# akashsengupta1997/HierarchicalProbabilistic3DHuman

Measured on AMD Instinct MI355X. Metric: images/sec end-to-end (num_samples=100), higher is better.
Workload: dtype f32

## Files before the change

hierarchicalprobabilistic3dhuman_amd/_capi.py:

```python
import contextlib
import ctypes
import os

import torch

_PKG_DIR = os.path.dirname(os.path.abspath(__file__))
LIB_PATH = os.path.join(_PKG_DIR, "libhps.so")
DEV_LIB_PATH = os.path.join(_PKG_DIR, "libhps_dev.so")

_c = ctypes
_P = _c.c_void_p
_I = _c.c_int

_PROTOTYPES = {
    "hps_version": [],
    "hps_last_error": [],
    "hps_stream_create_cu_partition": [_I, _I, _c.POINTER(_P)],
    "hps_stream_destroy": [_P],
    "hps_smpl_pose_prep": [_P, _P, _I, _P, _I, _P, _P, _P, _P, _I, _P, _I, _I, _P, _P, _P, _I, _P],
    "hps_smpl_blend": [_P, _P, _P, _P, _I, _I, _I, _I, _I, _I, _P],
    "hps_smpl_lbs": [_P, _I, _P, _P, _P, _I, _I, _P, _P, _I, _I, _P],
    "hps_smpl_mesh_fused": [_P, _P, _P, _P, _P, _P, _I, _I, _P, _P, _I, _I, _I, _I, _I, _P],
    "hps_smpl_mesh_fused_picks": [_P, _P, _P, _P, _P, _P, _I, _I, _P, _P, _I, _I, _I, _I, _I, _P, _P, _I, _P],
    "hps_smpl_mesh_fused_shared_shape": [_P] * 8 + [_I, _I, _P] + [_I] * 5 + [_P, _P, _I, _P],
    "hps_smpl_split_bf16x3_bytes": [_I, _I],
    "hps_smpl_split_bf16x3_mesh_tile": [],
    "hps_smpl_split_bf16x3": [_P, _I, _I, _I, _I, _P, _P],
    "hps_smpl_mesh_fused_shared_shape_bf16x3": [_P] * 8 + [_I, _I, _P] + [_I] * 4 + [_P, _P, _I, _P],
    "hps_smpl_v_shaped": [_P, _I, _P, _I, _P, _P, _I, _I, _P],
    "hps_smpl_mesh_fused_np": [_I],
    "hps_smpl_lbs_backward": [_P, _I, _P, _P, _P, _I, _I, _P, _P, _I, _P, _P, _P, _P, _P, _P, _I, _I, _P],
    "hps_smpl_blend_backward": [_P, _P, _P, _P, _I, _I, _I, _I, _I, _P],
    "hps_smpl_pose_prep_backward": [_P, _P, _I, _P, _I, _P, _P, _P, _P, _I, _P, _P, _I, _P, _I, _P, _P, _P, _I, _P],
    "hps_smpl_joints": [_P, _P, _P, _P, _P, _I, _I, _P, _P, _I, _I, _P],
    "hps_vertex_uncertainty": [_P, _P, _I, _I, _I, _P],
    "hps_joints_and_uncertainty": [_P, _P, _P, _P, _P, _I, _I, _P, _P, _I, _I, _P, _P, _I, _I, _I, _P],
    "hps_query_workspace": [_I, _c.c_int64, _c.c_int64, _c.c_int64],
    "hps_mf_sample": [_P, _P, _P, _P, _P, _I, _I, _I, _I, _c.c_float, _c.c_float, _P, _P, _P, _c.c_uint64,
                      _c.c_int64, _P, _I, _P, _P, _P, _P],
    "hps_infer_assemble": [_P, _P, _P, _P, _P, _P, _P, _I, _I, _I, _I, _P],
    "hps_quat_to_rotmat": [_P, _P, _I, _P],
    "hps_rot6d_to_rotmat": [_P, _P, _I, _P],
    "hps_batch_rodrigues": [_P, _P, _I, _P],
    "hps_linear": [_P, _I, _P, _P, _P, _P, _I, _I, _I, _I, _I, _P],
    "hps_head_trunk": [_P] + [_I] + [_P] * 14 + [_I] * 7 + [_P],
    "hps_head_joint_level": [_P, _I, _I, _P, _I, _P, _P, _P, _P, _P, _P, _P, _P, _P, _c.c_float, _P, _P, _I, _I, _P],
    "hps_head_joint_level_svd": [_P, _I, _I, _P, _I, _P, _P, _P, _P, _P, _P, _P, _P, _P, _c.c_float, _P, _P, _P, _P, _I, _I, _I, _P],
    "hps_svd3_packed": [_P, _P, _I, _I, _P],
    "hps_host_svd3_emulated": [_P, _P, _I, _I],
    "hps_host_svd_flavor": [],
    "hps_host_svd3_packed": [_P, _P, _I, _I],
    "hps_host_bind_lapack": [_c.c_char_p],
    "hps_head_svd_finish": [_P, _P, _I, _P, _P, _P, _P, _P, _P, _I, _I, _P],
    "hps_canny_edges": [_P, _P, _I, _P, _P, _P, _P, _P, _P, _I, _I, _I, _I, _c.c_float, _I, _P],
    "hps_canny_edge_map": [_P, _P, _I, _P, _c.c_int64, _I, _I, _I, _I, _c.c_float, _I, _P],
    "hps_proxy_rep": [_P, _P, _P, _P, _I, _I, _I, _I, _c.c_float, _P],
    "hps_pointset_errors": [_P, _P, _I, _I, _I, _I, _P, _P, _P, _P, _P],
    "hps_heatmaps_to_joints2d": [_P, _P, _P, _I, _I, _I, _c.c_float, _P],
    "hps_sample_joints2d_error": [_P, _P, _I, _P, _P, _P, _c.c_float, _P, _I, _I, _P],
    "hps_conv2d_bn_act_pad": [_P, _P, _P, _P, _P, _P, _I, _I, _I, _I, _I, _I, _I, _I, _I, _I, _I, _I, _I, _I, _I, _P, _P],
    "hps_conv2d_bn_act_pad_down": [_P] * 9 + [_I] * 14 + [_P, _P],
    "hps_conv3x3_winograd": [_P, _P, _P, _P, _P, _P, _I, _I, _I, _I, _I, _I, _I, _I, _P, _P],
    "hps_conv3x3_winograd_workspace": [_I, _I, _I, _I, _I],
    "hps_stem_phase_frames_bytes": [_I, _I, _I],
    "hps_stem_phase_split": [_P, _P, _I, _I, _I, _I, _P],
    "hps_proxy_rep_phase_frames": [_P, _P, _P, _P, _I, _I, _I, _I, _c.c_float, _P],
    "hps_stem_winograd": [_P, _P, _P, _P, _P, _I, _I, _I, _I, _I, _P],
    "hps_stem_pool_side_bytes": [_I, _I, _I],
    "hps_stem_winograd_pooled": [_P, _P, _P, _P, _P, _P, _I, _I, _I, _I, _I, _P],
    "hps_stem_winograd_pooled_nchw": [_P, _P, _P, _P, _P, _P, _I, _I, _I, _I, _I, _P],
    "hps_sums_f64": [_P, _P, _P, _I, _c.c_double, _P, _P, _P, _P],
    "hps_sizeof_enc_op": [],
    "hps_encoder_run": [_P, _I, _P],
    "hps_head_pose_levels": [_P, _I, _I, _P, _P, _I, _P, _P, _P, _P, _P, _P, _P, _P, _P, _c.c_float, _P, _P, _P, _P, _P, _P,
                             _P, _P, _I, _I, _I, _I, _P],
    "hps_nchw_to_padded_nhwc": [_P, _P, _I, _I, _I, _I, _I, _P],
    "hps_nchw_to_padded_nhwc_generic": [_P, _P, _I, _I, _I, _I, _I, _I, _I, _P],
    "hps_maxpool3x3s2_pad": [_P, _P, _I, _I, _I, _I, _I, _P],
    "hps_global_avgpool_pad": [_P, _P, _I, _I, _I, _I, _I, _P],
    "hps_mf_log_norm_const": [_P, _I, _P, _P, _P, _P],
    "hps_mf_nll": [_P, _P, _P, _P, _P, _I, _c.c_double, _P, _P, _P, _P, _P],
    "hps_mf_loss_forward": [_P, _P, _P, _P],
    "hps_mf_loss_backward": [_P, _P, _P, _P],
    "hps_head_forward_refine": [_P, _I] + [_P] * 9 + [_I] + [_P] * 6 + [_c.c_float] + [_P] * 13 + [_I] * 7 + [_P],
    "hps_head_pose_levels_backward": [_P, _I, _I, _P, _P, _I] + [_P] * 21 + [_I, _I, _I, _P],
    "hps_head_pose_levels_backward_factors": [_P, _I, _I, _P, _P, _I] + [_P] * 23 + [_I, _I, _I, _P],
    "hps_mf_sample_keep_quat": [_P, _P, _P, _I, _I, _I, _I, _c.c_float, _c.c_float, _P, _P, _P, _c.c_uint64, _c.c_int64, _I, _P, _P, _P, _P],
    "hps_mf_sample_backward": [_P, _P, _P, _P, _P, _P, _P, _P, _I, _I, _I, _c.c_float, _P, _P, _P, _P],
    "hps_head_trunk_backward": [_P, _I] + [_P] * 20 + [_I] * 7 + [_P],
    "hps_rot6d_to_rotmat_backward": [_P, _P, _P, _I, _P],
    "hps_conv_wgrad": [_P] * 4 + [_I] * 12 + [_P],
    "hps_conv_wgrad_slice_pixels": [_I, _I],
    "hps_conv_wgrad_workspace": [_I] * 9,
    "hps_conv_dgrad": [_P] * 4 + [_I] * 12 + [_P],
    "hps_relu_gate_pad": [_P] * 4 + [_I] * 6 + [_P],
    "hps_relu_gate_workspace": [_I] * 4,
    "hps_maxpool3x3s2_backward": [_P] * 3 + [_I] * 5 + [_P],
    "hps_global_avgpool_backward": [_P] * 2 + [_I] * 5 + [_P],
    "hps_bn_batch_stats": [_P] * 4 + [_I] * 5 + [_P],
    "hps_bn_batch_stats_workspace": [_I] * 4,
    "hps_bn_train_fold": [_P] * 5 + [_c.c_double, _c.c_double, _c.c_longlong] + [_P] * 5 + [_I, _P],
    "hps_bn_apply_act_pad": [_P] * 5 + [_I] * 7 + [_P],
    "hps_bn_train_backward_sums": [_P] * 7 + [_I] * 7 + [_P],
    "hps_bn_train_backward_sums_workspace": [_I] * 4,
    "hps_bn_train_backward_dz": [_P] * 7 + [_I] * 7 + [_P],
    "hps_seg_bbox_affine": [_P, _c.c_int64, _P, _I, _I, _I, _I, _c.c_float, _P, _P, _P, _P, _P, _P],
    "hps_train_crop_augment": [_P, _c.c_int64, _P, _P, _P, _P, _I, _I, _I, _I, _I, _P, _P, _P, _P, _P],
    "hps_train_joints2d": [_P, _P, _P, _P, _P, _I, _I, _c.c_float, _I, _I, _P, _P, _P, _P, _P],
}
_RESTYPES = {"hps_last_error": _c.c_char_p, "hps_smpl_split_bf16x3_bytes": _c.c_size_t, "hps_query_workspace": _c.c_int64, "hps_conv3x3_winograd_workspace": _c.c_size_t,
             "hps_stem_phase_frames_bytes": _c.c_size_t, "hps_stem_pool_side_bytes": _c.c_size_t,
             "hps_conv_wgrad_workspace": _c.c_size_t, "hps_relu_gate_workspace": _c.c_size_t,
             "hps_bn_batch_stats_workspace": _c.c_size_t, "hps_bn_train_backward_sums_workspace": _c.c_size_t}

EXPORTED_SYMBOLS = tuple(_PROTOTYPES)

_lib = None
_dev_lib = None
_use_dev = False


class EncOp(_c.Structure):
    _fields_ = [("kind", _I), ("x", _P), ("w", _P), ("scale", _P), ("shift", _P), ("residual", _P), ("y", _P),
                ("splitk_ws", _P)] + [(n, _I) for n in ("B", "H", "W", "ipad", "Cin", "Cout", "KH", "KW", "stride", "pad", "opad",
                                                       "relu", "row_mode", "variant", "ksplit")] + [
                    ("w_down", _P), ("scale_down", _P), ("shift_down", _P), ("y_down", _P)]


class MfLossArgs(_c.Structure):
    _fields_ = [("struct_bytes", _I), ("reduction", _I)] + [
        (n, _c.c_int64) for n in ("n_pose", "shape_B", "n_shape", "j2d_B", "Ns", "K", "n_glob", "n_verts", "n_joints3d")] + [
        ("img_wh", _c.c_double), ("overreg", _c.c_double), ("weights", _c.c_double * 6)] + [
        (n, _P) for n in ("pose_F", "pose_U", "pose_S", "pose_V", "shape_loc", "shape_scale", "joints2d", "glob_rotmats", "verts",
                          "joints3d", "t_pose_rotmats", "t_shape", "t_joints2d", "t_joints2d_vis", "t_glob_rotmats", "t_verts",
                          "t_joints3d", "g_pose_F", "g_pose_S", "g_shape_loc", "g_shape_scale", "g_joints2d", "g_glob_rotmats",
                          "g_verts", "g_joints3d")]


MF_REDUCTION_MEAN, MF_REDUCTION_SUM = 0, 1
ENC_RELAYOUT, ENC_CONV, ENC_MAXPOOL, ENC_AVGPOOL, ENC_CONV_WINOGRAD, ENC_STEM_SPLIT, ENC_STEM_WINOGRAD, ENC_RELAYOUT_GENERIC = 0, 1, 2, 3, 4, 5, 6, 7
ENC_STEM_WINOGRAD_POOLED, ENC_STEM_WINOGRAD_POOLED_NCHW, ENC_CONV_DOWN = 8, 9, 10
ENC_ENTRY = {kind: (entry, tuple(fields.split())) for kind, entry, fields in (
    (ENC_RELAYOUT, "hps_nchw_to_padded_nhwc", "x y B Cin H W opad"),
    (ENC_RELAYOUT_GENERIC, "hps_nchw_to_padded_nhwc_generic", "x y B Cin Cout H W KW opad"),
    (ENC_CONV, "hps_conv2d_bn_act_pad", "x w scale shift residual y B H W ipad Cin Cout KH KW stride pad opad relu row_mode variant ksplit splitk_ws"),
    (ENC_CONV_DOWN, "hps_conv2d_bn_act_pad_down", "x w scale shift y w_down scale_down shift_down y_down B H W ipad Cin Cout KH KW stride pad opad "
                                                  "relu variant ksplit splitk_ws"),
    (ENC_CONV_WINOGRAD, "hps_conv3x3_winograd", "x w scale shift residual y B H W ipad Cin Cout opad relu splitk_ws"),
    (ENC_STEM_SPLIT, "hps_stem_phase_split", "x y B Cin H W"),
    (ENC_STEM_WINOGRAD, "hps_stem_winograd", "x w scale shift y B H W opad relu"),
    (ENC_STEM_WINOGRAD_POOLED, "hps_stem_winograd_pooled", "x w scale shift y splitk_ws B H W opad relu"),
    (ENC_STEM_WINOGRAD_POOLED_NCHW, "hps_stem_winograd_pooled_nchw", "x w scale shift y splitk_ws B H W opad relu"),
    (ENC_MAXPOOL, "hps_maxpool3x3s2_pad", "x y B H W Cin opad"),
    (ENC_AVGPOOL, "hps_global_avgpool_pad", "x y B H W Cin ipad"))}
SVD_HOST, SVD_DEVICE, SVD_DEVICE_FMA = 0, 1, 2
SVD_ROUNDING_REFERENCE, SVD_ROUNDING_FMA = 0, 1
HEAD_WIDE_WORKGROUPS = 0x100


class HpsError(RuntimeError):
    pass


def _open(path, prototypes, what):
    if not os.path.exists(path):
        raise HpsError(
            "%s is missing (%s). Build it with `python -m hierarchicalprobabilistic3dhuman_amd.build` "
            "(hipcc --offload-arch=gfx950). There is no CPU fallback for this path." % (what, path))
    lib = ctypes.CDLL(path)
    for name, argtypes in prototypes.items():
        fn = getattr(lib, name)
        fn.argtypes = argtypes
        fn.restype = _RESTYPES.get(name, _I)
    torch_cpu = os.path.join(os.path.dirname(torch.__file__), "lib", "libtorch_cpu.so")
    if os.path.exists(torch_cpu):
        lib.hps_host_bind_lapack(torch_cpu.encode())
    return lib


def load(dev=False):
    global _lib, _dev_lib
    if dev:
        if _dev_lib is None:
            _dev_lib = _open(DEV_LIB_PATH, dict(_PROTOTYPES, **_dev_prototypes()), "libhps_dev.so")
        return _dev_lib
    if _lib is None:
        _lib = _open(LIB_PATH, _PROTOTYPES, "libhps.so")
    return _lib


def _dev_prototypes():
    import importlib.util
    path = os.path.join(os.path.dirname(_PKG_DIR), "tests", "devlib.py")
    if not os.path.exists(path):
        raise HpsError("libhps_dev.so is test infrastructure: its prototypes live in tests/devlib.py, which is missing (%s)" % path)
    spec = importlib.util.spec_from_file_location("hps_tests_devlib_prototypes", path)
    mod = importlib.util.module_from_spec(spec)
    spec.loader.exec_module(mod)
    return mod.DEV_PROTOTYPES


@contextlib.contextmanager
def dev_library():
    global _use_dev
    prev, _use_dev = _use_dev, True
    try:
        yield load(dev=True)
    finally:
        _use_dev = prev


def require_device(t, what="tensor"):
    if not isinstance(t, torch.Tensor) or not t.is_cuda:
        raise HpsError(
            "%s must live on a HIP (MI355X) device; this package has no CPU path "
            "(the CPU oracle under oracle/ is test infrastructure only)" % what)
    if t.device.index != torch.cuda.current_device():
        raise HpsError("%s lives on cuda:%d but the current device is cuda:%d; call torch.cuda.set_device(%d) "
                       "(or use `with torch.cuda.device(...)`) before calling into libhps"
                       % (what, t.device.index, torch.cuda.current_device(), t.device.index))


def ptr(t, dtype=torch.float32, what="tensor"):
    if t is None:
        return None
    require_device(t, what)
    if t.dtype != dtype:
        raise HpsError("%s: expected %s, got %s" % (what, dtype, t.dtype))
    if not t.is_contiguous():
        raise HpsError("%s must be contiguous" % what)
    return _P(t.data_ptr())


def iptr(t, what="index tensor"):
    return ptr(t, torch.int32, what)


def stream():
    return _P(torch.cuda.current_stream().cuda_stream)


def cu_partition_stream(first_cu, num_cus):
    s = _P()
    call("hps_stream_create_cu_partition", int(first_cu), int(num_cus), _c.byref(s))
    if not _partition_streams:
        import atexit
        atexit.register(_destroy_partition_streams)
    _partition_streams.append(s.value)
    return torch.cuda.ExternalStream(s.value)


_partition_streams = []


def _destroy_partition_streams():
    try:
        if torch.cuda.is_available():
            torch.cuda.synchronize()
        lib = load()
        while _partition_streams:
            lib.hps_stream_destroy(_P(_partition_streams.pop()))
    except Exception:
        pass


_svd_flavor = None
_svd_flavor_exact = None


def svd_flavor():
    global _svd_flavor, _svd_flavor_exact
    if _svd_flavor is None:
        fl = load(dev=_use_dev).hps_host_svd_flavor()
        _svd_flavor_exact = fl in (SVD_ROUNDING_REFERENCE, SVD_ROUNDING_FMA)
        if not _svd_flavor_exact:
            import warnings
            warnings.warn("libhps: neither rounding flavour of the in-kernel 3x3 SVD reproduces this host's LAPACK sgesdd bit for "
                          "bit; using reference rounding (expect about one differently signed singular-vector pair in 10^4 "
                          "matrices relative to torch.svd on this host; svd_mode='host' is exact)")
            fl = SVD_ROUNDING_REFERENCE
        _svd_flavor = fl
    return _svd_flavor


def svd_flavor_is_exact():
    svd_flavor()
    return bool(_svd_flavor_exact)


def call(name, *args):
    lib = load(dev=_use_dev)
    rc = getattr(lib, name)(*args)
    if rc != 0:
        msg = lib.hps_last_error()
        raise HpsError("%s failed (code %d): %s" % (name, rc, msg.decode() if msg else ""))


def issue_enc_op(op):
    entry, fields = ENC_ENTRY[op.kind]
    call(entry, *[getattr(op, f) for f in fields], stream())


def run_enc_ops(ops, first, count, composite=True):
    if not composite:
        for i in range(first, first + count):
            issue_enc_op(ops[i])
    elif first == 0:
        call("hps_encoder_run", ops, count, stream())
    else:
        call("hps_encoder_run", _c.cast(_c.byref(ops, first * _c.sizeof(EncOp)), _c.POINTER(EncOp)), count, stream())


WS_CONV_SPLITK, WS_SMPL_MP, WS_SMPL_XT, WS_SMPL_A, WS_SMPL_VPOSED, WS_HEAD_F, WS_HEAD_USV = range(7)
WS_MF_LOSS = 8
WS_SMPL_LBS_BWD, WS_SMPL_BLEND_BWD = 9, 10
WS_HEAD_LEVELS_BWD, WS_HEAD_TRUNK_BWD = 11, 12
WS_SEG_BBOX = 13


def query_workspace(what, d0=0, d1=0, d2=0):
    n = load(dev=_use_dev).hps_query_workspace(int(what), int(d0), int(d1), int(d2))
    if n < 0:
        raise HpsError("hps_query_workspace(%d, %d, %d, %d) failed" % (what, d0, d1, d2))
    return int(n)


def f32c(t):
    if t.dtype != torch.float32:
        t = t.float()
    return t.contiguous()
```

hierarchicalprobabilistic3dhuman_amd/csrc/composite.hip:

```cpp
#include <vector>

#include "hps_common.h"

using namespace hps;

extern "C" int hps_sizeof_enc_op(void) { return (int)sizeof(hps_enc_op); }

extern "C" int hps_encoder_run(const hps_enc_op* ops, int n_ops, hps_stream_t stream) {
    if (!ops && n_ops > 0) return bad_arg("hps_encoder_run: null op list");
    for (int i = 0; i < n_ops; ++i) {
        const hps_enc_op& o = ops[i];
        int rc;
        switch (o.kind) {
            case HPS_ENC_RELAYOUT:
                rc = hps_nchw_to_padded_nhwc(o.x, o.y, o.B, o.Cin, o.H, o.W, o.opad, stream);
                break;
            case HPS_ENC_RELAYOUT_GENERIC:
                rc = hps_nchw_to_padded_nhwc_generic(o.x, o.y, o.B, o.Cin, o.Cout, o.H, o.W, o.KW, o.opad, stream);
                break;
            case HPS_ENC_CONV:
                rc = hps_conv2d_bn_act_pad(o.x, o.w, o.scale, o.shift, o.residual, o.y, o.B, o.H, o.W, o.ipad, o.Cin, o.Cout,
                                           o.KH, o.KW, o.stride, o.pad, o.opad, o.relu, o.row_mode, o.variant, o.ksplit,
                                           o.splitk_ws, stream);
                break;
            case HPS_ENC_CONV_DOWN:
                rc = hps_conv2d_bn_act_pad_down(o.x, o.w, o.scale, o.shift, o.y, o.w_down, o.scale_down, o.shift_down, o.y_down, o.B, o.H,
                                                o.W, o.ipad, o.Cin, o.Cout, o.KH, o.KW, o.stride, o.pad, o.opad, o.relu, o.variant, o.ksplit,
                                                o.splitk_ws, stream);
                break;
            case HPS_ENC_CONV_WINOGRAD:
                rc = hps_conv3x3_winograd(o.x, o.w, o.scale, o.shift, o.residual, o.y, o.B, o.H, o.W, o.ipad, o.Cin, o.Cout, o.opad,
                                          o.relu, o.splitk_ws, stream);
                break;
            case HPS_ENC_STEM_SPLIT:
                rc = hps_stem_phase_split(o.x, o.y, o.B, o.Cin, o.H, o.W, stream);
                break;
            case HPS_ENC_STEM_WINOGRAD:
                rc = hps_stem_winograd(o.x, o.w, o.scale, o.shift, o.y, o.B, o.H, o.W, o.opad, o.relu, stream);
                break;
            case HPS_ENC_STEM_WINOGRAD_POOLED:
                rc = hps_stem_winograd_pooled(o.x, o.w, o.scale, o.shift, o.y, o.splitk_ws, o.B, o.H, o.W, o.opad, o.relu, stream);
                break;
            case HPS_ENC_STEM_WINOGRAD_POOLED_NCHW:
                rc = hps_stem_winograd_pooled_nchw(o.x, o.w, o.scale, o.shift, o.y, o.splitk_ws, o.B, o.H, o.W, o.opad, o.relu, stream);
                break;
            case HPS_ENC_MAXPOOL:
                rc = hps_maxpool3x3s2_pad(o.x, o.y, o.B, o.H, o.W, o.Cin, o.opad, stream);
                break;
            case HPS_ENC_AVGPOOL:
                rc = hps_global_avgpool_pad(o.x, o.y, o.B, o.H, o.W, o.Cin, o.ipad, stream);
                break;
            default:
                return bad_arg("hps_encoder_run: unknown op kind");
        }
        if (rc != HPS_OK) return rc;
    }
    return HPS_OK;
}

extern "C" int hps_head_pose_levels(const float* embed, int embed_dim, int hidden, const int32_t* level_joints,
                                    const int32_t* level_sizes_host, int n_levels, const int32_t* anc_ptr,
                                    const int32_t* anc_idx, const float* const* w1t_ptrs, const float* const* b1_ptrs,
                                    const float* const* w2_ptrs, const float* const* b2_ptrs, float* u_proper,
                                    float* s_proper, float* mode, float delta_i_weight, float* pose_f, float* pose_u,
                                    float* pose_s, float* pose_v, float* f_level_dev, float* usv_level_dev,
                                    float* f_host_pinned, float* usv_host_pinned, int B, int num_body_joints,
                                    int svd_threads, int svd_mode, hps_stream_t stream) {
    if (!embed || !level_joints || !level_sizes_host) return bad_arg("hps_head_pose_levels: null pointer");
    const int wide = svd_mode & HPS_HEAD_WIDE_WORKGROUPS;
    svd_mode &= ~HPS_HEAD_WIDE_WORKGROUPS;
    if (svd_mode == HPS_SVD_DEVICE || svd_mode == HPS_SVD_DEVICE_FMA) {
        const int flavor = (svd_mode == HPS_SVD_DEVICE_FMA ? HPS_SVD_ROUNDING_FMA : HPS_SVD_ROUNDING_REFERENCE) | wide;
        int first_d = 0;
        for (int l = 0; l < n_levels; ++l) {
            const int n_level = level_sizes_host[l];
            const int rc = hps_head_joint_level_svd(embed, embed_dim, hidden, level_joints + first_d, n_level, anc_ptr, anc_idx,
                                                    w1t_ptrs, b1_ptrs, w2_ptrs, b2_ptrs, u_proper, s_proper, mode, delta_i_weight,
                                                    pose_f, pose_u, pose_s, pose_v, B, num_body_joints, flavor, stream);
            if (rc != HPS_OK) return rc;
            first_d += n_level;
        }
        return HPS_OK;
    }
    if (svd_mode != HPS_SVD_HOST) return bad_arg("hps_head_pose_levels: svd_mode");
    if (!f_level_dev || !usv_level_dev || !f_host_pinned || !usv_host_pinned)
        return bad_arg("hps_head_pose_levels: the host-LAPACK mode needs the staging buffers");
    hipStream_t s = (hipStream_t)stream;
    int first = 0;
    for (int l = 0; l < n_levels; ++l) {
        const int n_level = level_sizes_host[l];
        const int32_t* ids = level_joints + first;
        const size_t count = (size_t)B * n_level;
        int rc = hps_head_joint_level(embed, embed_dim, hidden, ids, n_level, anc_ptr, anc_idx, w1t_ptrs, b1_ptrs, w2_ptrs,
                                      b2_ptrs, u_proper, s_proper, mode, delta_i_weight, pose_f, f_level_dev, B,
                                      num_body_joints, stream);
        if (rc != HPS_OK) return rc;
        hipError_t e = hipMemcpyAsync(f_host_pinned, f_level_dev, count * 9 * sizeof(float), hipMemcpyDeviceToHost, s);
        if (e == hipSuccess) e = hipStreamSynchronize(s);
        if (e != hipSuccess) {
            set_error("hps_head_pose_levels: %s", hipGetErrorString(e));
            return (int)e;
        }
        rc = hps_host_svd3_packed(f_host_pinned, usv_host_pinned, (int)count, svd_threads);
        if (rc != HPS_OK) return rc;
        e = hipMemcpyAsync(usv_level_dev, usv_host_pinned, count * 21 * sizeof(float), hipMemcpyHostToDevice, s);
        if (e != hipSuccess) {
            set_error("hps_head_pose_levels: %s", hipGetErrorString(e));
            return (int)e;
        }
        rc = hps_head_svd_finish(usv_level_dev, ids, n_level, pose_u, pose_s, pose_v, u_proper, s_proper, mode, B,
                                 num_body_joints, stream);
        if (rc != HPS_OK) return rc;
        first += n_level;
    }
    return HPS_OK;
}
```

hierarchicalprobabilistic3dhuman_amd/csrc/head.hip:

```cpp
#include "hps_common.h"
#include "svd3_gesdd.h"

namespace hps {

__device__ __forceinline__ float elu1(float x) { return x > 0.0f ? x : expm1f(x); }


constexpr int TB = 8;
constexpr int LCOLS = 16;
constexpr int LKS = 16;

template <int ROWS>
__device__ __forceinline__ void dot_slice(const float* __restrict__ w, size_t ldw, const float* xs, int k_lo, int k_hi,
                                          float (&acc)[ROWS]) {
    int k = k_lo;
    for (; k + 8 <= k_hi; k += 8) {
        float wv[8];
#pragma unroll
        for (int u = 0; u < 8; ++u) wv[u] = w[(size_t)(k + u) * ldw];
#pragma unroll
        for (int u = 0; u < 8; ++u) {
            const float4* xr = reinterpret_cast<const float4*>(xs + (k + u) * ROWS);
#pragma unroll
            for (int q = 0; q < ROWS / 4; ++q) {
                const float4 xv = xr[q];
                acc[q * 4 + 0] += xv.x * wv[u]; acc[q * 4 + 1] += xv.y * wv[u];
                acc[q * 4 + 2] += xv.z * wv[u]; acc[q * 4 + 3] += xv.w * wv[u];
            }
        }
    }
    for (; k < k_hi; ++k) {
        const float wv = w[(size_t)k * ldw];
        const float4* xr = reinterpret_cast<const float4*>(xs + k * ROWS);
#pragma unroll
        for (int q = 0; q < ROWS / 4; ++q) {
            const float4 xv = xr[q];
            acc[q * 4 + 0] += xv.x * wv; acc[q * 4 + 1] += xv.y * wv;
            acc[q * 4 + 2] += xv.z * wv; acc[q * 4 + 3] += xv.w * wv;
        }
    }
}

struct TrunkSplit {
    float* loc; float* scale; float* glob; float* cam;
    int nsh, ng, nc;
};

__global__ __launch_bounds__(256) void linear_kernel(const float* __restrict__ x, int ldx, const float* __restrict__ x2, int ldx2, int K1,
                                                     const float* __restrict__ wt,
                                                     const float* __restrict__ bias, const float* __restrict__ addend,
                                                     float* __restrict__ out, int ldo, int B, int K, int N, int act, TrunkSplit split) {
    __builtin_amdgcn_s_setprio(3);
    extern __shared__ __attribute__((aligned(16))) float smem[];
    float* xs = smem;
    float* red = smem + (size_t)((K * TB + 3) & ~3);
    const int b0 = blockIdx.y * TB;
    const int col = threadIdx.x % LCOLS, ks = threadIdx.x / LCOLS;
    const int n = blockIdx.x * LCOLS + col;

    for (int i = threadIdx.x; i < K * TB; i += 256) {
        const int r = i / K, k = i % K;
        xs[k * TB + r] = (b0 + r < B) ? (k < K1 ? x[(size_t)(b0 + r) * ldx + k] : x2[(size_t)(b0 + r) * ldx2 + (k - K1)]) : 0.0f;
    }
    __syncthreads();

    float acc[TB];
#pragma unroll
    for (int r = 0; r < TB; ++r) acc[r] = 0.0f;
    const int kchunk = ceil_div(K, LKS);
    const int k_lo = min(K, ks * kchunk), k_hi = min(K, k_lo + kchunk);
    if (n < N) dot_slice<TB>(wt + n, (size_t)N, xs, k_lo, k_hi, acc);
#pragma unroll
    for (int r = 0; r < TB; ++r) red[(ks * TB + r) * LCOLS + col] = acc[r];
    __syncthreads();
    if (threadIdx.x < TB * LCOLS) {
        const int r = threadIdx.x / LCOLS, c = threadIdx.x % LCOLS;
        const int nn = blockIdx.x * LCOLS + c;
        if (nn < N && b0 + r < B) {
            float v = 0.0f;
#pragma unroll
            for (int q = 0; q < LKS; ++q) v += red[(q * TB + r) * LCOLS + c];
            v += bias[nn] + (addend ? addend[nn] : 0.0f);
            if (act == HPS_ACT_ELU) v = elu1(v);
            else if (act == HPS_ACT_RELU) v = fmaxf(v, 0.0f);
            out[(size_t)(b0 + r) * ldo + nn] = v;
            if (split.loc) {
                const size_t b = (size_t)(b0 + r);
                const int h = split.nsh;
                if (nn < h) split.loc[b * h + nn] = v;
                else if (nn < 2 * h) split.scale[b * h + (nn - h)] = expf(v);
                else if (nn < 2 * h + split.ng) split.glob[b * split.ng + (nn - 2 * h)] = v;
                else split.cam[b * split.nc + (nn - 2 * h - split.ng)] = v;
            }
        }
    }
}

#pragma clang fp contract(off)
__device__ __forceinline__ float det3_unfused(const float* m) {
    return m[0] * (m[4] * m[8] - m[5] * m[7]) - m[1] * (m[3] * m[8] - m[5] * m[6]) +
           m[2] * (m[3] * m[7] - m[4] * m[6]);
}
__device__ __forceinline__ void mat3_mul_bt_unfused(const float* a, const float* b, float* c) {
#pragma unroll
    for (int i = 0; i < 3; ++i)
#pragma unroll
        for (int j = 0; j < 3; ++j)
            c[i * 3 + j] = a[i * 3 + 0] * b[j * 3 + 0] + a[i * 3 + 1] * b[j * 3 + 1] + a[i * 3 + 2] * b[j * 3 + 2];
}
__device__ __forceinline__ void proper_svd_store(float* U, const float* S, float* V, size_t o, float* __restrict__ pose_u,
                                                 float* __restrict__ pose_s, float* __restrict__ pose_v, float* u_proper,
                                                 float* s_proper, float* mode) {
#pragma unroll
    for (int e = 0; e < 9; ++e) { pose_u[o * 9 + e] = U[e]; pose_v[o * 9 + e] = V[e]; }
#pragma unroll
    for (int e = 0; e < 3; ++e) pose_s[o * 3 + e] = S[e];
    const float dU = det3_unfused(U), dV = det3_unfused(V);
    U[2] *= dU; U[5] *= dU; U[8] *= dU;
    V[2] *= dV; V[5] *= dV; V[8] *= dV;
    float Mo[9];
    mat3_mul_bt_unfused(U, V, Mo);
#pragma unroll
    for (int e = 0; e < 9; ++e) { u_proper[o * 9 + e] = U[e]; mode[o * 9 + e] = Mo[e]; }
    s_proper[o * 3 + 0] = S[0];
    s_proper[o * 3 + 1] = S[1];
    s_proper[o * 3 + 2] = S[2] * (dU * dV);
}
#pragma clang fp contract(fast)

template <int HID, bool DEVSVD, int NT, int TBL>
__device__ __forceinline__ void joint_level_body(
    float* smem, const int joint, const int slot, const int n_slots, const int b0,
    const float* __restrict__ embed, int embed_dim,
    const int32_t* __restrict__ anc_ptr, const int32_t* __restrict__ anc_idx, const float* const* __restrict__ w1t_ptrs,
    const float* const* __restrict__ b1_ptrs, const float* const* __restrict__ w2_ptrs,
    const float* const* __restrict__ b2_ptrs, float* u_proper, float* s_proper,
    float* mode, float delta_i_weight, float* __restrict__ pose_f, float* __restrict__ f_level,
    float* __restrict__ pose_u, float* __restrict__ pose_s, float* __restrict__ pose_v, int B, int NJ, int svd_flavor,
    int* published = nullptr) {
    constexpr int KS = NT / HID;
    constexpr int PARTS = NT >= 9 * TBL * 8 ? 8 : 4;
    static_assert(NT % HID == 0 && TBL % 4 == 0 && NT >= 9 * TBL * PARTS && KS * HID >= 9, "joint_level_kernel: shape");
    const int a_lo = anc_ptr[joint], P = anc_ptr[joint + 1] - a_lo;
    const int in_dim = embed_dim + 21 * P;
    float* xs = smem;
    float* hs = smem + (size_t)((in_dim * TBL + 3) & ~3);
    float* red = hs + HID * TBL;

    int* s_anc = reinterpret_cast<int*>(red);
    if ((int)threadIdx.x < P) s_anc[threadIdx.x] = anc_idx[a_lo + threadIdx.x];
    __syncthreads();
    auto source = [&](int i, bool& live) -> const float* {
        const int r = i / in_dim, k = i - r * in_dim;
        const int b = min(b0 + r, B - 1);
        live = b0 + r < B && i < in_dim * TBL;
        if (k < embed_dim) return embed + (size_t)b * embed_dim + k;
        int t = k - embed_dim;
        if (t < 9 * P) return u_proper + ((size_t)b * NJ + s_anc[t / 9]) * 9 + t % 9;
        t -= 9 * P;
        if (t < 3 * P) return s_proper + ((size_t)b * NJ + s_anc[t / 3]) * 3 + t % 3;
        t -= 3 * P;
        return mode + ((size_t)b * NJ + s_anc[max(0, min(t / 9, P - 1))]) * 9 + t % 9;
    };
    for (int i0 = threadIdx.x; i0 < in_dim * TBL; i0 += 4 * NT) {
        float v[4];
        bool live[4];
#pragma unroll
        for (int q = 0; q < 4; ++q) v[q] = *source(min(i0 + q * NT, in_dim * TBL - 1), live[q]);
#pragma unroll
        for (int q = 0; q < 4; ++q) {
            const int i = i0 + q * NT;
            if (i < in_dim * TBL) {
                const int r = i / in_dim, k = i - r * in_dim;
                xs[k * TBL + r] = (b0 + r < B) ? v[q] : 0.0f;
            }
        }
    }
    __syncthreads();

    const int n = threadIdx.x % HID, ks = threadIdx.x / HID;
    float acc[TBL];
#pragma unroll
    for (int r = 0; r < TBL; ++r) acc[r] = 0.0f;
    const int kchunk = ceil_div(in_dim, KS);
    const int k_lo = min(in_dim, ks * kchunk), k_hi = min(in_dim, k_lo + kchunk);
    dot_slice<TBL>(w1t_ptrs[joint] + n, (size_t)HID, xs, k_lo, k_hi, acc);
#pragma unroll
    for (int r = 0; r < TBL; ++r) red[(ks * TBL + r) * HID + n] = acc[r];
    __syncthreads();
    for (int i = threadIdx.x; i < HID * TBL; i += NT) {
        const int r = i / HID, c = i % HID;
        float v = b1_ptrs[joint][c];
#pragma unroll
        for (int q = 0; q < KS; ++q) v += red[(q * TBL + r) * HID + c];
        hs[c * TBL + r] = elu1(v);
    }
    __syncthreads();

    if (threadIdx.x < 9 * TBL * PARTS) {
        const int part = threadIdx.x % PARTS, o = threadIdx.x / PARTS;
        const int e = o / TBL, r = o % TBL;
        const float* w2 = w2_ptrs[joint] + (size_t)e * HID;
        float v = 0.0f;
        for (int k = part; k < HID; k += PARTS) v += w2[k] * hs[k * TBL + r];
#pragma unroll
        for (int m = 1; m < PARTS; m <<= 1) v += __shfl_xor(v, m);
        if (part == 0) {
            v += b2_ptrs[joint][e];
            if (e % 4 == 0) v += delta_i_weight;
            if (b0 + r < B) {
                pose_f[((size_t)(b0 + r) * NJ + joint) * 9 + e] = v;
                if (f_level) f_level[((size_t)(b0 + r) * n_slots + slot) * 9 + e] = v;
            }
            if (DEVSVD) red[r * 9 + e] = v;
        }
    }
    if (DEVSVD) {
        static_assert(NT / 64 >= TBL, "one wave per image of the tile");
        __syncthreads();
        const int r = threadIdx.x >> 6;
        if ((threadIdx.x & 63) == 0 && r < TBL && b0 + r < B) {
            float F[9], U[9], S[3], V[9];
#pragma unroll
            for (int e = 0; e < 9; ++e) F[e] = red[r * 9 + e];
            gesdd3::svd3(svd_flavor, F, U, S, V);
            proper_svd_store(U, S, V, (size_t)(b0 + r) * NJ + joint, pose_u, pose_s, pose_v, u_proper, s_proper, mode);
            if (published) __hip_atomic_fetch_add(published, 1, __ATOMIC_RELEASE, __HIP_MEMORY_SCOPE_AGENT);
        }
    }
}

template <int HID, bool DEVSVD, int NT, int TBL>
__global__ __launch_bounds__(NT) void joint_level_kernel(
    const float* __restrict__ embed, int embed_dim, const int32_t* __restrict__ joint_ids,
    const int32_t* __restrict__ anc_ptr, const int32_t* __restrict__ anc_idx, const float* const* __restrict__ w1t_ptrs,
    const float* const* __restrict__ b1_ptrs, const float* const* __restrict__ w2_ptrs,
    const float* const* __restrict__ b2_ptrs, float* u_proper, float* s_proper,
    float* mode, float delta_i_weight, float* __restrict__ pose_f, float* __restrict__ f_level,
    float* __restrict__ pose_u, float* __restrict__ pose_s, float* __restrict__ pose_v, int B, int NJ, int svd_flavor) {
    __builtin_amdgcn_s_setprio(3);
    extern __shared__ __attribute__((aligned(16))) float smem[];
    joint_level_body<HID, DEVSVD, NT, TBL>(smem, joint_ids[blockIdx.x], (int)blockIdx.x, (int)gridDim.x, (int)blockIdx.y * TBL, embed,
                                           embed_dim, anc_ptr, anc_idx, w1t_ptrs, b1_ptrs, w2_ptrs, b2_ptrs, u_proper, s_proper, mode,
                                           delta_i_weight, pose_f, f_level, pose_u, pose_s, pose_v, B, NJ, svd_flavor);
}

#ifdef HPS_DEV_BUILD
struct LevelTable {
    int n_levels;
    int first[HPS_HEAD_MAX_LEVELS];
    int size[HPS_HEAD_MAX_LEVELS];
};
template <int HID, int NT, int TBL>
__global__ __launch_bounds__(NT) void joint_levels_fused_kernel(
    const float* __restrict__ embed, int embed_dim, const int32_t* __restrict__ level_joints, const LevelTable lv,
    const int32_t* __restrict__ anc_ptr, const int32_t* __restrict__ anc_idx, const float* const* __restrict__ w1t_ptrs,
    const float* const* __restrict__ b1_ptrs, const float* const* __restrict__ w2_ptrs,
    const float* const* __restrict__ b2_ptrs, float* u_proper, float* s_proper,
    float* mode, float delta_i_weight, float* __restrict__ pose_f,
    float* __restrict__ pose_u, float* __restrict__ pose_s, float* __restrict__ pose_v, int B, int NJ, int svd_flavor, int* sync) {
    __builtin_amdgcn_s_setprio(3);
    extern __shared__ __attribute__((aligned(16))) float smem[];
    const int slot = blockIdx.x, tile = blockIdx.y;
    int* cnt = sync + (size_t)tile * (HPS_HEAD_MAX_LEVELS + 1);
    const int n_live = min(TBL, B - tile * TBL);
    for (int l = 0; l < lv.n_levels; ++l) {
        if (l > 0) {
            if (threadIdx.x == 0) {
                while (__hip_atomic_load(cnt + (l - 1), __ATOMIC_RELAXED, __HIP_MEMORY_SCOPE_AGENT) < lv.size[l - 1] * n_live) __builtin_amdgcn_s_sleep(1);
            }
            __syncthreads();
            __builtin_amdgcn_fence(__ATOMIC_ACQUIRE, "agent");
        }
        if (slot < lv.size[l])
            joint_level_body<HID, true, NT, TBL>(smem, level_joints[lv.first[l] + slot], slot, lv.size[l], tile * TBL, embed, embed_dim,
                                                 anc_ptr, anc_idx, w1t_ptrs, b1_ptrs, w2_ptrs, b2_ptrs, u_proper, s_proper, mode,
                                                 delta_i_weight, pose_f, nullptr, pose_u, pose_s, pose_v, B, NJ, svd_flavor, cnt + l);
    }
    __syncthreads();
    if (threadIdx.x == 0) {
        const int arrived = __hip_atomic_fetch_add(cnt + HPS_HEAD_MAX_LEVELS, 1, __ATOMIC_ACQ_REL, __HIP_MEMORY_SCOPE_AGENT);
        if (arrived == (int)gridDim.x - 1) {
            for (int l = 0; l <= HPS_HEAD_MAX_LEVELS; ++l) __hip_atomic_store(cnt + l, 0, __ATOMIC_RELAXED, __HIP_MEMORY_SCOPE_AGENT);
        }
    }
}

#endif

__global__ void svd_finish_kernel(const float* __restrict__ usv, const int32_t* __restrict__ joint_ids, int n_level,
                                  float* __restrict__ pose_u, float* __restrict__ pose_s, float* __restrict__ pose_v,
                                  float* __restrict__ u_proper, float* __restrict__ s_proper, float* __restrict__ mode,
                                  int B, int NJ) {
    const int i = blockIdx.x * blockDim.x + threadIdx.x;
    if (i >= B * n_level) return;
    const int b = i / n_level, joint = joint_ids[i % n_level];
    const size_t o = (size_t)b * NJ + joint;
    const float* src = usv + (size_t)i * 21;
    float U[9], V[9], S[3];
#pragma unroll
    for (int e = 0; e < 9; ++e) { U[e] = src[e]; V[e] = src[12 + e]; }
#pragma unroll
    for (int e = 0; e < 3; ++e) S[e] = src[9 + e];
    proper_svd_store(U, S, V, o, pose_u, pose_s, pose_v, u_proper, s_proper, mode);
}

__global__ void svd3_packed_kernel(const float* __restrict__ f, float* __restrict__ usv, int n, int svd_flavor) {
    const int i = blockIdx.x * blockDim.x + threadIdx.x;
    if (i >= n) return;
    float F[9], U[9], S[3], V[9];
#pragma unroll
    for (int e = 0; e < 9; ++e) F[e] = f[(size_t)i * 9 + e];
    gesdd3::svd3(svd_flavor, F, U, S, V);
    float* o = usv + (size_t)i * 21;
#pragma unroll
    for (int e = 0; e < 9; ++e) { o[e] = U[e]; o[12 + e] = V[e]; }
    o[9] = S[0]; o[10] = S[1]; o[11] = S[2];
}

}

using namespace hps;

static int launch_linear(const char* who, const float* x, int ldx, const float* x2, int ldx2, int K1, const float* wt, const float* bias,
                         const float* addend, float* out, int ldo, int B, int K, int N, int act, TrunkSplit split, hps_stream_t stream) {
    size_t lds = ((size_t)((K * TB + 3) & ~3) + LKS * TB * LCOLS) * sizeof(float);
    if (lds > 64 * 1024) { set_error("%s: K=%d too large for the LDS tile", who, K); return HPS_E_UNSUPPORTED; }
    hipLaunchKernelGGL(linear_kernel, dim3(ceil_div(N, LCOLS), ceil_div(B, TB)), dim3(256), lds, (hipStream_t)stream, x,
                       ldx, x2, ldx2, K1, wt, bias, addend, out, ldo, B, K, N, act, split);
    return check_launch(who);
}

extern "C" int hps_linear(const float* x, int ldx, const float* wt, const float* bias, const float* addend, float* out,
                          int ldo, int B, int K, int N, int act, hps_stream_t stream) {
    if (!x || !wt || !bias || !out) return bad_arg("hps_linear: null pointer");
    if (K <= 0 || N <= 0 || ldx < K || ldo < N) return bad_arg("hps_linear: dims");
    if (B <= 0) return HPS_OK;
    return launch_linear("hps_linear", x, ldx, nullptr, 0, K, wt, bias, addend, out, ldo, B, K, N, act, TrunkSplit{}, stream);
}

extern "C" int hps_head_trunk(const float* feats, int ldf, const float* fc1_wt, const float* fc1_b, const float* sgc_wt,
                              const float* sgc_b, const float* sgc_add, const float* embed_wt, const float* embed_b, float* x_ws,
                              float* sgc_out, float* embed, float* shape_loc, float* shape_scale, float* glob, float* cam, int B,
                              int num_feats, int hidden, int num_shape, int num_glob, int num_cam, int embed_dim,
                              hps_stream_t stream) {
    if (!feats || !fc1_wt || !fc1_b || !sgc_wt || !sgc_b || !embed_wt || !embed_b || !x_ws || !sgc_out || !embed || !shape_loc ||
        !shape_scale || !glob || !cam)
        return bad_arg("hps_head_trunk: null pointer");
    if (num_feats <= 0 || hidden <= 0 || num_shape <= 0 || num_glob <= 0 || num_cam <= 0 || embed_dim <= 0 || ldf < num_feats)
        return bad_arg("hps_head_trunk: dims");
    if (B <= 0) return HPS_OK;
    const int nt = 2 * num_shape + num_glob + num_cam;
    int rc = launch_linear("hps_head_trunk", feats, ldf, nullptr, 0, num_feats, fc1_wt, fc1_b, nullptr, x_ws, hidden, B, num_feats,
                           hidden, HPS_ACT_ELU, TrunkSplit{}, stream);
    if (rc != HPS_OK) return rc;
    TrunkSplit sp{shape_loc, shape_scale, glob, cam, num_shape, num_glob, num_cam};
    rc = launch_linear("hps_head_trunk", x_ws, hidden, nullptr, 0, hidden, sgc_wt, sgc_b, sgc_add, sgc_out, nt, B, hidden, nt,
                       HPS_ACT_NONE, sp, stream);
    if (rc != HPS_OK) return rc;
    return launch_linear("hps_head_trunk", feats, ldf, sgc_out, nt, num_feats, embed_wt, embed_b, nullptr, embed, embed_dim, B,
                         num_feats + nt, embed_dim, HPS_ACT_ELU, TrunkSplit{}, stream);
}

static int joint_level_launch(const float* embed, int embed_dim, int hidden, const int32_t* joint_ids, int n_level,
                              const int32_t* anc_ptr, const int32_t* anc_idx, const float* const* w1t_ptrs,
                              const float* const* b1_ptrs, const float* const* w2_ptrs, const float* const* b2_ptrs,
                              float* u_proper, float* s_proper, float* mode, float delta_i_weight, float* pose_f,
                              float* f_level, float* pose_u, float* pose_s, float* pose_v, int B, int num_body_joints,
                              int svd_flavor, hps_stream_t stream) {
    const bool devsvd = pose_u != nullptr;
    const bool wide = devsvd && (svd_flavor & HPS_HEAD_WIDE_WORKGROUPS) != 0;
    svd_flavor &= ~HPS_HEAD_WIDE_WORKGROUPS;
    if (devsvd && svd_flavor != HPS_SVD_ROUNDING_REFERENCE && svd_flavor != HPS_SVD_ROUNDING_FMA)
        return bad_arg("hps_head_joint_level_svd: svd_flavor");
    if (!embed || !joint_ids || !anc_ptr || !anc_idx || !w1t_ptrs || !b1_ptrs || !w2_ptrs || !b2_ptrs || !u_proper ||
        !s_proper || !mode || !pose_f || (devsvd && (!pose_s || !pose_v)))
        return bad_arg("hps_head_joint_level: null pointer");
    if (hidden != 128) { set_error("hps_head_joint_level: hidden=%d unsupported (128 = EMBED_DIM/2)", hidden); return HPS_E_UNSUPPORTED; }
    if (B <= 0 || n_level <= 0) return HPS_OK;
    constexpr int NT = 256, TBL = 4;
    const int max_in = embed_dim + 21 * num_body_joints;
    size_t lds = ((size_t)((max_in * TBL + 3) & ~3) + 128 * TBL + (NT / 128) * TBL * 128) * sizeof(float);
    if (lds > 64 * 1024) { set_error("hps_head_joint_level: embed_dim=%d too large", embed_dim); return HPS_E_UNSUPPORTED; }
    constexpr int NTW = 1024;
    const size_t ldsw = ((size_t)((max_in * TBL + 3) & ~3) + 128 * TBL + (NTW / 128) * TBL * 128) * sizeof(float);
    if (wide && ldsw <= 64 * 1024) {
        hipLaunchKernelGGL((joint_level_kernel<128, true, NTW, TBL>), dim3(n_level, ceil_div(B, TBL)), dim3(NTW), ldsw, (hipStream_t)stream,
                           embed, embed_dim, joint_ids, anc_ptr, anc_idx, w1t_ptrs, b1_ptrs, w2_ptrs, b2_ptrs, u_proper,
                           s_proper, mode, delta_i_weight, pose_f, f_level, pose_u, pose_s, pose_v, B, num_body_joints, svd_flavor);
    } else if (devsvd)
        hipLaunchKernelGGL((joint_level_kernel<128, true, NT, TBL>), dim3(n_level, ceil_div(B, TBL)), dim3(NT), lds, (hipStream_t)stream,
                           embed, embed_dim, joint_ids, anc_ptr, anc_idx, w1t_ptrs, b1_ptrs, w2_ptrs, b2_ptrs, u_proper,
                           s_proper, mode, delta_i_weight, pose_f, f_level, pose_u, pose_s, pose_v, B, num_body_joints, svd_flavor);
    else
        hipLaunchKernelGGL((joint_level_kernel<128, false, NT, TBL>), dim3(n_level, ceil_div(B, TBL)), dim3(NT), lds, (hipStream_t)stream,
                           embed, embed_dim, joint_ids, anc_ptr, anc_idx, w1t_ptrs, b1_ptrs, w2_ptrs, b2_ptrs, u_proper,
                           s_proper, mode, delta_i_weight, pose_f, f_level, pose_u, pose_s, pose_v, B, num_body_joints, svd_flavor);
    return check_launch("hps_head_joint_level");
}

extern "C" int hps_head_joint_level(const float* embed, int embed_dim, int hidden, const int32_t* joint_ids,
                                    int n_level, const int32_t* anc_ptr, const int32_t* anc_idx,
                                    const float* const* w1t_ptrs, const float* const* b1_ptrs,
                                    const float* const* w2_ptrs, const float* const* b2_ptrs, const float* u_proper,
                                    const float* s_proper, const float* mode, float delta_i_weight, float* pose_f,
                                    float* f_level, int B, int num_body_joints, hps_stream_t stream) {
    return joint_level_launch(embed, embed_dim, hidden, joint_ids, n_level, anc_ptr, anc_idx, w1t_ptrs, b1_ptrs, w2_ptrs, b2_ptrs,
                              const_cast<float*>(u_proper), const_cast<float*>(s_proper), const_cast<float*>(mode),
                              delta_i_weight, pose_f, f_level, nullptr, nullptr, nullptr, B, num_body_joints, 0, stream);
}

extern "C" int hps_head_joint_level_svd(const float* embed, int embed_dim, int hidden, const int32_t* joint_ids,
                                        int n_level, const int32_t* anc_ptr, const int32_t* anc_idx,
                                        const float* const* w1t_ptrs, const float* const* b1_ptrs,
                                        const float* const* w2_ptrs, const float* const* b2_ptrs, float* u_proper,
                                        float* s_proper, float* mode, float delta_i_weight, float* pose_f, float* pose_u,
                                        float* pose_s, float* pose_v, int B, int num_body_joints, int svd_flavor,
                                        hps_stream_t stream) {
    if (!pose_u) return bad_arg("hps_head_joint_level_svd: null pointer");
    return joint_level_launch(embed, embed_dim, hidden, joint_ids, n_level, anc_ptr, anc_idx, w1t_ptrs, b1_ptrs, w2_ptrs, b2_ptrs,
                              u_proper, s_proper, mode, delta_i_weight, pose_f, nullptr, pose_u, pose_s, pose_v, B,
                              num_body_joints, svd_flavor, stream);
}

#ifdef HPS_DEV_BUILD
extern "C" int hps_dev_head_pose_levels_fused(const float* embed, int embed_dim, int hidden, const int32_t* level_joints,
                                          const int32_t* level_sizes_host, int n_levels, const int32_t* anc_ptr,
                                          const int32_t* anc_idx, const float* const* w1t_ptrs, const float* const* b1_ptrs,
                                          const float* const* w2_ptrs, const float* const* b2_ptrs, float* u_proper,
                                          float* s_proper, float* mode, float delta_i_weight, float* pose_f, float* pose_u,
                                          float* pose_s, float* pose_v, int B, int num_body_joints, int svd_flavor,
                                          int32_t* sync_ws, hps_stream_t stream) {
    const bool wide = (svd_flavor & HPS_HEAD_WIDE_WORKGROUPS) != 0;
    svd_flavor &= ~HPS_HEAD_WIDE_WORKGROUPS;
    if (svd_flavor != HPS_SVD_ROUNDING_REFERENCE && svd_flavor != HPS_SVD_ROUNDING_FMA) return bad_arg("hps_dev_head_pose_levels_fused: svd_flavor");
    if (!embed || !level_joints || !level_sizes_host || !anc_ptr || !anc_idx || !w1t_ptrs || !b1_ptrs || !w2_ptrs || !b2_ptrs ||
        !u_proper || !s_proper || !mode || !pose_f || !pose_u || !pose_s || !pose_v || !sync_ws)
        return bad_arg("hps_dev_head_pose_levels_fused: null pointer");
    if (hidden != 128) { set_error("hps_dev_head_pose_levels_fused: hidden=%d unsupported (128 = EMBED_DIM/2)", hidden); return HPS_E_UNSUPPORTED; }
    if (n_levels < 1 || n_levels > HPS_HEAD_MAX_LEVELS) return bad_arg("hps_dev_head_pose_levels_fused: n_levels");
    if (B <= 0) return HPS_OK;
    LevelTable lv;
    lv.n_levels = n_levels;
    int widest = 0, first = 0;
    for (int l = 0; l < HPS_HEAD_MAX_LEVELS; ++l) {
        lv.first[l] = first;
        lv.size[l] = l < n_levels ? level_sizes_host[l] : 0;
        if (lv.size[l] < 0) return bad_arg("hps_dev_head_pose_levels_fused: level size");
        first += lv.size[l];
        widest = lv.size[l] > widest ? lv.size[l] : widest;
    }
    if (widest == 0) return HPS_OK;
    constexpr int NT = 256, NTW = 1024, TBL = 4;
    const int tiles = ceil_div(B, TBL);
    int dev = 0, cus = 0;
    if (hipGetDevice(&dev) != hipSuccess || hipDeviceGetAttribute(&cus, hipDeviceAttributeMultiprocessorCount, dev) != hipSuccess) cus = 0;
    if ((long)widest * tiles > (long)cus) {
        set_error("hps_dev_head_pose_levels_fused: %d x %d workgroups do not fit the device's %d CUs at once; use hps_head_pose_levels", widest, tiles, cus);
        return HPS_E_UNSUPPORTED;
    }
    const int max_in = embed_dim + 21 * num_body_joints;
    const size_t lds = ((size_t)((max_in * TBL + 3) & ~3) + 128 * TBL + (NT / 128) * TBL * 128) * sizeof(float);
    const size_t ldsw = ((size_t)((max_in * TBL + 3) & ~3) + 128 * TBL + (NTW / 128) * TBL * 128) * sizeof(float);
    if (lds > 64 * 1024) { set_error("hps_dev_head_pose_levels_fused: embed_dim=%d too large", embed_dim); return HPS_E_UNSUPPORTED; }
    if (wide && ldsw <= 64 * 1024)
        hipLaunchKernelGGL((joint_levels_fused_kernel<128, NTW, TBL>), dim3(widest, tiles), dim3(NTW), ldsw, (hipStream_t)stream, embed, embed_dim,
                           level_joints, lv, anc_ptr, anc_idx, w1t_ptrs, b1_ptrs, w2_ptrs, b2_ptrs, u_proper, s_proper, mode, delta_i_weight,
                           pose_f, pose_u, pose_s, pose_v, B, num_body_joints, svd_flavor, sync_ws);
    else
        hipLaunchKernelGGL((joint_levels_fused_kernel<128, NT, TBL>), dim3(widest, tiles), dim3(NT), lds, (hipStream_t)stream, embed, embed_dim,
                           level_joints, lv, anc_ptr, anc_idx, w1t_ptrs, b1_ptrs, w2_ptrs, b2_ptrs, u_proper, s_proper, mode, delta_i_weight,
                           pose_f, pose_u, pose_s, pose_v, B, num_body_joints, svd_flavor, sync_ws);
    return check_launch("hps_dev_head_pose_levels_fused");
}

#endif

extern "C" int hps_svd3_packed(const float* f, float* usv, int n, int svd_flavor, hps_stream_t stream) {
    if (!f || !usv) return bad_arg("hps_svd3_packed: null pointer");
    if (svd_flavor != HPS_SVD_ROUNDING_REFERENCE && svd_flavor != HPS_SVD_ROUNDING_FMA) return bad_arg("hps_svd3_packed: svd_flavor");
    if (n <= 0) return HPS_OK;
    hipLaunchKernelGGL(svd3_packed_kernel, dim3(ceil_div(n, 64)), dim3(64), 0, (hipStream_t)stream, f, usv, n, svd_flavor);
    return check_launch("hps_svd3_packed");
}

extern "C" int hps_head_svd_finish(const float* usv_level, const int32_t* joint_ids, int n_level, float* pose_u,
                                   float* pose_s, float* pose_v, float* u_proper, float* s_proper, float* mode, int B,
                                   int num_body_joints, hps_stream_t stream) {
    if (!usv_level || !pose_u || !pose_s || !pose_v || !joint_ids || !u_proper || !s_proper || !mode)
        return bad_arg("hps_head_svd_finish: null pointer");
    if (B <= 0 || n_level <= 0) return HPS_OK;
    hipLaunchKernelGGL(svd_finish_kernel, dim3(ceil_div(B * n_level, 128)), dim3(128), 0, (hipStream_t)stream, usv_level,
                       joint_ids, n_level, pose_u, pose_s, pose_v, u_proper, s_proper, mode, B, num_body_joints);
    return check_launch("hps_head_svd_finish");
}
```

hierarchicalprobabilistic3dhuman_amd/csrc/mesh_epilogue.h:

```cpp
#pragma once

#include <type_traits>

#include "hps_common.h"

namespace hps {

typedef float f32x16 __attribute__((ext_vector_type(16)));

constexpr int MESH_PANEL = 64;

struct MeshGrid {
    int tiles_m_per_xcd;
    unsigned blocks;
};
inline MeshGrid mesh_grid(int tiles_m, int n_panels) {
    const int per_xcd = tiles_m >= 8 ? ceil_div(tiles_m, 8) : 0;
    return {per_xcd, (unsigned)(per_xcd ? per_xcd * 8 * n_panels : tiles_m * n_panels)};
}
__device__ __forceinline__ bool mesh_block(int tiles_m, int tiles_m_per_xcd, int& tile_m, int& panel) {
    const int xcd = blockIdx.x & 7, local = blockIdx.x >> 3;
    tile_m = tiles_m_per_xcd ? (local % tiles_m_per_xcd) * 8 + xcd : (int)blockIdx.x % tiles_m;
    panel = tiles_m_per_xcd ? local / tiles_m_per_xcd : (int)blockIdx.x / tiles_m;
    return tile_m < tiles_m;
}

template <int K>
struct MeshLane {
    int lane, wave, kl, il, wm, wn;
    int v, vc;
    bool live_v;
    int idx[K];
    float w[K];
    f3 vt, vtb;
    int split, split_lane;
    bool many;
    int pick;
};

template <int K, int MG, bool VS, bool PICK>
__device__ __forceinline__ MeshLane<K> mesh_lane(int panel, int m0, int V, const int32_t* __restrict__ w_idx,
                                                 const float* __restrict__ w_val, const float* __restrict__ v_template,
                                                 const int32_t* __restrict__ group_rows, const int32_t* __restrict__ pick_slot) {
    MeshLane<K> L;
    const int tid = threadIdx.x;
    L.lane = tid & 63;
    L.wave = __builtin_amdgcn_readfirstlane(tid >> 6);
    L.kl = L.lane >> 5;
    L.il = L.lane & 31;
    L.wm = L.wave >> 1;
    L.wn = L.wave & 1;
    L.v = panel * MESH_PANEL + L.wn * 32 + L.il;
    L.live_v = L.v < V;
    L.vc = L.live_v ? L.v : V - 1;
#pragma unroll
    for (int k = 0; k < K; ++k) {
        L.idx[k] = w_idx[(size_t)L.vc * K + k] * 12;
        L.w[k] = w_val[(size_t)L.vc * K + k];
    }
    const f3* vtp = reinterpret_cast<const f3*>(v_template);
    L.split = 32;
    L.many = false;
    if (VS) {
        const int32_t* gr = group_rows + 3 * __builtin_amdgcn_readfirstlane((m0 + L.wm * 32) >> 5);
        const int row_a = gr[0], row_b = gr[1];
        L.split = gr[2];
        L.vt = vtp[(size_t)row_a * V + L.vc];
        L.vtb = vtp[(size_t)row_b * V + L.vc];
#pragma unroll
        for (int h = 0; h < MG; ++h) L.many |= group_rows[3 * (m0 / 32 + h) + 2] < 0;
    } else {
        L.vt = vtp[L.vc];
        L.vtb = L.vt;
    }
    L.split_lane = L.split - 4 * L.kl;
    L.pick = PICK && L.live_v ? pick_slot[L.vc] : -1;
    return L;
}

__device__ __forceinline__ void mesh_keep_acc(const f32x16 (&acc)[3], f3* verts) {
    float t = 0.f;
#pragma unroll
    for (int r = 0; r < 16; ++r) t += acc[0][r] + acc[1][r] + acc[2][r];
    if (t == 12345.678f) verts[0].x = t;
}

enum MeshEpi { EPI_ALL = 0, EPI_NO_SKIN, EPI_NO_A_DMA, EPI_NO_STORES };

template <int K, int JC, int MG, bool HAS_T, bool PICK, bool VS, int EPI = EPI_ALL>
__device__ __forceinline__ void mesh_epilogue(float* smem, const MeshLane<K>& L, const f32x16 (&acc)[3], int m0, int M, int V, int J,
                                              const float* __restrict__ a, const float* __restrict__ transl,
                                              const float* __restrict__ v_template, const int32_t* __restrict__ mesh_row,
                                              f3* __restrict__ verts, f3* __restrict__ picked, int n_picked) {
    typedef __attribute__((address_space(3))) void* lptr_t;
    const unsigned lds0 = (unsigned)(size_t)(lptr_t)(smem);
    const int a_stride = JC ? JC * 12 : J * 12;
    const int half_bytes = 16 * a_stride * 4;
    const int slot0 = L.wm * 16 + 4 * L.kl;
    int aoff[K];
#pragma unroll
    for (int k = 0; k < K; ++k) aoff[k] = slot0 * a_stride + L.idx[k];
    char* const vbase = reinterpret_cast<char*>(verts) + (size_t)(m0 + L.wm * 32) * V * 12;
    const unsigned voff = ((unsigned)(4 * L.kl) * (unsigned)V + (unsigned)L.v) * 12u;
    char* const pbase = PICK ? reinterpret_cast<char*>(picked) + (size_t)(m0 + L.wm * 32) * n_picked * 12 : nullptr;
    const unsigned poff = PICK ? ((unsigned)(4 * L.kl) * (unsigned)n_picked + (unsigned)max(L.pick, 0)) * 12u : 0u;
    auto epilogue = [&](auto many_c) __attribute__((always_inline)) {
        constexpr bool MANY = decltype(many_c)::value;
#pragma unroll
        for (int pass = 0; pass < 2; ++pass) {
            __syncthreads();
#pragma unroll
            for (int h = 0; h < MG; ++h) {
                const int mh = m0 + 32 * h + 16 * pass;
                const int valid = max(0, min(16, M - mh)) * a_stride * 4;
                const float* a_src = a + (size_t)mh * a_stride;
                for (int piece = L.wave; piece * 1024 < half_bytes; piece += 2 * MG) {
                    const int off = piece * 1024 + L.lane * 16;
                    if (off < valid && EPI != EPI_NO_A_DMA) lds_dma16((unsigned)off, a_src, lds0 + (unsigned)(h * half_bytes + piece * 1024));
                }
            }
            asm volatile("s_waitcnt vmcnt(0)" ::: "memory");
            __syncthreads();
#pragma unroll
            for (int q = 0; q < 8; ++q) {
                const int r = 8 * pass + q;
                const int dr = (r & 3) + 8 * (r >> 2);
                const int ds = (q & 3) + 8 * (q >> 2);
                const int m = m0 + L.wm * 32 + 4 * L.kl + dr;
                float tx = 0.f, ty = 0.f, tz = 0.f;
                if (HAS_T) {
                    const float* t = transl + (size_t)min(m, M - 1) * 3;
                    tx = t[0]; ty = t[1]; tz = t[2];
                }
                f3 base = L.vt;
                if (VS && !MANY) {
                    const bool first = dr < L.split_lane;
                    base.x = first ? L.vt.x : L.vtb.x; base.y = first ? L.vt.y : L.vtb.y; base.z = first ? L.vt.z : L.vtb.z;
                }
                if (VS && MANY) base = reinterpret_cast<const f3*>(v_template)[(size_t)mesh_row[min(m, M - 1)] * V + L.vc];
                f3 pv;
                pv.x = base.x + acc[0][r]; pv.y = base.y + acc[1][r]; pv.z = base.z + acc[2][r];
                f3 o;
                if (EPI == EPI_NO_SKIN) {
                    o = pv;
                } else {
                    int ao[K];
#pragma unroll
                    for (int k = 0; k < K; ++k) ao[k] = aoff[k] + ds * a_stride;
                    o = skin_vertex<K>(smem, ao, L.w, pv, tx, ty, tz);
                }
                asm volatile("" :: "v"(o.x), "v"(o.y), "v"(o.z));
                if (EPI == EPI_NO_STORES) {
                    if (o.x == 12345.678f) *reinterpret_cast<f3*>(vbase + (size_t)dr * V * 12 + voff) = o;
                    continue;
                }
                if (L.live_v && m < M) *reinterpret_cast<f3*>(vbase + (size_t)dr * V * 12 + voff) = o;
                if (PICK && L.pick >= 0 && m < M) *reinterpret_cast<f3*>(pbase + (size_t)dr * n_picked * 12 + poff) = o;
            }
        }
    };
    if (VS && L.many) epilogue(std::true_type());
    else epilogue(std::false_type());
}

}
```

hierarchicalprobabilistic3dhuman_amd/csrc/mesh_fused.hip:

```cpp

#include "mesh_epilogue.h"

namespace hps {

constexpr int FM = 64;
constexpr int FV = MESH_PANEL;
constexpr int FN = 3 * FV;
constexpr int FBK = 16;
constexpr int FT = 256;
constexpr int FW = FT / 64;
constexpr int F_CHUNK_FLOATS = FBK * (FM + FN);
constexpr int F_XP = FBK * FM / 256;
constexpr int F_BP = FBK * FN / 256;
static_assert(F_XP == FW && F_BP % FW == 0, "DMA pieces must divide evenly over the waves");

template <int K, int ABL, int JC, bool HAS_T, int TAIL = FBK / 2, int ST = 2, bool PICK = false, bool VS = false>
__global__ __launch_bounds__(FT, 4) void mesh_fused_kernel(
    const float* __restrict__ xt, const float* __restrict__ bmat_p, const float* __restrict__ v_template,
    const float* __restrict__ a, const int32_t* __restrict__ w_idx, const float* __restrict__ w_val, int J,
    const float* __restrict__ transl, f3* __restrict__ verts, int M, int V, int kp, int mp, int np, int tiles_m,
    int tiles_m_per_xcd, const int32_t* __restrict__ pick_slot, f3* __restrict__ picked, int n_picked,
    const int32_t* __restrict__ mesh_row, const int32_t* __restrict__ group_rows) {
    typedef __attribute__((address_space(3))) void* lptr_t;
    extern __shared__ __attribute__((aligned(16))) float smem[];

    int tile_m, panel;
    if (!mesh_block(tiles_m, tiles_m_per_xcd, tile_m, panel)) return;
    const int m0 = tile_m * FM;
    const MeshLane<K> L = mesh_lane<K, FM / 32, VS, PICK>(panel, m0, V, w_idx, w_val, v_template, group_rows, pick_slot);
    const int lane = L.lane, wave = L.wave, kl = L.kl, il = L.il, wm = L.wm, wn = L.wn;

    unsigned b_off[F_BP / FW];
#pragma unroll
    for (int j = 0; j < F_BP / FW; ++j) {
        const int f = 256 * (wave + FW * j) + 4 * lane;
        b_off[j] = (unsigned)(((f / FN) * np + (f % FN)) * 4);
    }
    unsigned x_off;
    {
        const int f = 256 * wave + 4 * lane;
        x_off = (unsigned)(((f / FM) * mp + (f % FM)) * 4);
    }
    const unsigned lds0 = (unsigned)(size_t)(lptr_t)(smem);
    const float* b_src = bmat_p + (size_t)panel * FN;
    const float* x_src = xt + m0;
    auto dma_chunk = [&](int buf) {
        const unsigned base = lds0 + (unsigned)buf * F_CHUNK_FLOATS * 4;
        lds_dma16(x_off, x_src, base + (unsigned)wave * 1024);
#pragma unroll
        for (int j = 0; j < F_BP / FW; ++j) lds_dma16(b_off[j], b_src, base + FBK * FM * 4 + (unsigned)(wave + FW * j) * 1024);
        b_src += (size_t)FBK * np;
        x_src += (size_t)FBK * mp;
    };
    auto dma_piece = [&](int p, int buf, const float* xs, const float* bs) {
        const unsigned base = lds0 + (unsigned)buf * F_CHUNK_FLOATS * 4;
        if (p == 0) lds_dma16(x_off, xs, base + (unsigned)wave * 1024);
        else lds_dma16(b_off[p - 1], bs, base + FBK * FM * 4 + (unsigned)(wave + FW * (p - 1)) * 1024);
    };

    f32x16 acc[3];
#pragma unroll
    for (int c = 0; c < 3; ++c)
#pragma unroll
        for (int r = 0; r < 16; ++r) acc[c][r] = 0.0f;

    const int nchunks = (kp + FBK - 1) / FBK;
    if (ABL != 4) {
        dma_chunk(0);
#pragma unroll
        for (int q = 1; q < ST - 1; ++q)
            if (q < nchunks) dma_chunk(q);
    }
    static_assert(1 + F_BP / FW == FBK / 4, "four DMA pieces per wave and chunk, one per two k-steps");
    constexpr int PIECES = 1 + F_BP / FW;
    auto do_chunk = [&](auto pairs_c, int c, bool more_in) __attribute__((always_inline)) {
        constexpr int PAIRS = decltype(pairs_c)::value;
        const bool more = ST == 2 ? more_in : (ABL != 4 && c + ST - 1 < nchunks);
        {
            const int younger = min(ST - 2, nchunks - 1 - c);
            if (ST >= 4 && younger >= 2) asm volatile("s_waitcnt vmcnt(%0)" ::"n"(2 * PIECES) : "memory");
            else if (ST >= 3 && younger >= 1) asm volatile("s_waitcnt vmcnt(%0)" ::"n"(PIECES) : "memory");
            else asm volatile("s_waitcnt vmcnt(0)" ::: "memory");
        }
        __syncthreads();
        constexpr bool burst = ABL == 5 && ST == 2;
        const float* nx_src = x_src;
        const float* nb_src = b_src;
        const int nbuf = ST == 2 ? (c + 1) & 1 : (c + ST - 1) % ST;
        if (more && burst) dma_chunk((c + 1) & 1);
        else if (more) { b_src += (size_t)FBK * np; x_src += (size_t)FBK * mp; }
        const float* sX = smem + (ST == 2 ? (c & 1) : c % ST) * F_CHUNK_FLOATS;
        const float* sB = sX + FBK * FM;
        float af[PAIRS], bx[PAIRS], by[PAIRS], bz[PAIRS];
#pragma unroll
        for (int k = 0; k < 2 * PAIRS; k += 2) {
            af[k / 2] = sX[(k + kl) * FM + wm * 32 + il];
            const float* brow = sB + (k + kl) * FN + wn * 32 + il;
            bx[k / 2] = brow[0]; by[k / 2] = brow[FV]; bz[k / 2] = brow[2 * FV];
        }
        __builtin_amdgcn_sched_barrier(0);
#pragma unroll
        for (int k = 0; k < PAIRS; ++k) {
            if (ABL == 2) {
                acc[0][0] += af[k] * bx[k]; acc[1][0] += af[k] * by[k]; acc[2][0] += af[k] * bz[k];
                continue;
            }
            acc[0] = __builtin_amdgcn_mfma_f32_32x32x2f32(af[k], bx[k], acc[0], 0, 0, 0);
            acc[1] = __builtin_amdgcn_mfma_f32_32x32x2f32(af[k], by[k], acc[1], 0, 0, 0);
            acc[2] = __builtin_amdgcn_mfma_f32_32x32x2f32(af[k], bz[k], acc[2], 0, 0, 0);
            if (more && !burst && (k & 1) == 0) {
                __builtin_amdgcn_sched_barrier(0);
                dma_piece(k / 2, nbuf, nx_src, nb_src);
                __builtin_amdgcn_sched_barrier(0);
            }
        }
    };
    for (int c = 0; c + 1 < nchunks; ++c) do_chunk(std::integral_constant<int, FBK / 2>(), c, ABL != 4);
    do_chunk(std::integral_constant<int, TAIL>(), nchunks - 1, false);

    if (ABL == 3) {
        mesh_keep_acc(acc, verts);
        return;
    }
    mesh_epilogue<K, JC, FM / 32, HAS_T, PICK, VS, ABL == 1 ? EPI_NO_SKIN : EPI_ALL>(smem, L, acc, m0, M, V, J, a, transl, v_template,
                                                                                       mesh_row, verts, picked, n_picked);
}

#ifdef HPS_DEV_BUILD
static size_t g_mesh_lds_floor = 0;
static int g_mesh_stages = 0;
#endif

template <int K, int ABL, int JC, bool HAS_T>
static int launch_fused_cfg(const float* xt, const float* bmat_p, const float* v_template, const float* a, const int32_t* w_idx,
                        const float* w_val, int J, const float* transl, float* verts, int M, int V, int kp, int mp, int np,
                        hipStream_t s, const int32_t* pick_slot = nullptr, float* picked = nullptr, int n_picked = 0,
                        const int32_t* mesh_row = nullptr, const int32_t* group_rows = nullptr) {
    size_t lds = (size_t)4 * max(2 * F_CHUNK_FLOATS, 32 * J * 12);
#ifdef HPS_DEV_BUILD
    if (g_mesh_lds_floor > lds) lds = g_mesh_lds_floor;
#endif
    const int tiles_m = ceil_div(M, FM), n_panels = ceil_div(V, FV);
    const bool few = tiles_m <= 2
#ifdef HPS_DEV_BUILD
                     && g_mesh_stages != 2
#endif
        ;
    const MeshGrid g = mesh_grid(tiles_m, n_panels);
    const int tail = (kp - FBK * ((kp + FBK - 1) / FBK - 1)) / 2;
    f3* pk = reinterpret_cast<f3*>(picked);
#define HPS_MESH_LAUNCH(...)                                                                                                       \
    do {                                                                                                                           \
        if (int rc = grant_lds<&mesh_fused_kernel<__VA_ARGS__>>(160 * 1024, "hps_smpl_mesh_fused")) return rc;                    \
        hipLaunchKernelGGL((mesh_fused_kernel<__VA_ARGS__>), dim3(g.blocks), dim3(FT), lds, s, xt, bmat_p, v_template, a, w_idx,   \
                           w_val, J, transl, reinterpret_cast<f3*>(verts), M, V, kp, mp, np, tiles_m, g.tiles_m_per_xcd,           \
                           pick_slot, pk, n_picked, mesh_row, group_rows);                                                         \
    } while (0)
    if constexpr (K == 4 && JC == 24 && ABL == 0 && !HAS_T) {
        if (group_rows) {
            if (tail != 8 || !pick_slot || !mesh_row) {
                set_error("hps_smpl_mesh_fused_shared_shape: exists for kp = 208 (SMPL's 207 pose rows) with the side output only");
                return HPS_E_UNSUPPORTED;
            }
            if (few) {
                lds = (size_t)4 * max(4 * F_CHUNK_FLOATS, 32 * J * 12);
                HPS_MESH_LAUNCH(K, ABL, JC, HAS_T, 8, 4, true, true);
            } else {
                HPS_MESH_LAUNCH(K, ABL, JC, HAS_T, 8, 2, true, true);
            }
            return check_launch("hps_smpl_mesh_fused_shared_shape");
        }
    }
    if (group_rows) {
        set_error("hps_smpl_mesh_fused_shared_shape: exists for K = 4, 24 joints, no translation");
        return HPS_E_UNSUPPORTED;
    }
    if constexpr (K == 4 && JC == 24 && ABL == 0) {
        if (tail == 5) {
            if (few) {
                lds = (size_t)4 * max(4 * F_CHUNK_FLOATS, 32 * J * 12);
                if (pick_slot) HPS_MESH_LAUNCH(K, ABL, JC, HAS_T, 5, 4, true);
                else HPS_MESH_LAUNCH(K, ABL, JC, HAS_T, 5, 4, false);
            } else {
                if (pick_slot) HPS_MESH_LAUNCH(K, ABL, JC, HAS_T, 5, 2, true);
                else HPS_MESH_LAUNCH(K, ABL, JC, HAS_T, 5, 2, false);
            }
            return check_launch("hps_smpl_mesh_fused");
        }
    }
    if (pick_slot) {
        set_error("hps_smpl_mesh_fused_picks: the side output exists for K = 4, 24 joints, kp = 218 (SMPL) only");
        return HPS_E_UNSUPPORTED;
    }
    HPS_MESH_LAUNCH(K, ABL, JC, HAS_T);
#undef HPS_MESH_LAUNCH
    return check_launch("hps_smpl_mesh_fused");
}

template <int K, int ABL = 0>
static int launch_fused(const float* xt, const float* bmat_p, const float* v_template, const float* a, const int32_t* w_idx,
                        const float* w_val, int J, const float* transl, float* verts, int M, int V, int kp, int mp, int np,
                        hipStream_t s, const int32_t* pick_slot = nullptr, float* picked = nullptr, int n_picked = 0,
                        const int32_t* mesh_row = nullptr, const int32_t* group_rows = nullptr) {
    if (J == 24 && !transl) return launch_fused_cfg<K, ABL, 24, false>(xt, bmat_p, v_template, a, w_idx, w_val, J, transl, verts, M, V, kp, mp, np, s, pick_slot, picked, n_picked, mesh_row, group_rows);
    if (group_rows) { set_error("hps_smpl_mesh_fused_shared_shape: 24 joints, no translation"); return HPS_E_UNSUPPORTED; }
    if (J == 24) return launch_fused_cfg<K, ABL, 24, true>(xt, bmat_p, v_template, a, w_idx, w_val, J, transl, verts, M, V, kp, mp, np, s, pick_slot, picked, n_picked);
    if (pick_slot) { set_error("hps_smpl_mesh_fused_picks: 24 joints only"); return HPS_E_UNSUPPORTED; }
    if constexpr (K == 4) {
        if (!transl) return launch_fused_cfg<K, ABL, 0, false>(xt, bmat_p, v_template, a, w_idx, w_val, J, transl, verts, M, V, kp, mp, np, s);
        return launch_fused_cfg<K, ABL, 0, true>(xt, bmat_p, v_template, a, w_idx, w_val, J, transl, verts, M, V, kp, mp, np, s);
    } else {
        set_error("hps_smpl_mesh_fused: K = %d is fused only for num_joints = 24 (use hps_smpl_blend + hps_smpl_lbs)", K);
        return HPS_E_UNSUPPORTED;
    }
}

}

using namespace hps;

extern "C" int hps_smpl_mesh_fused_np(int V) { return V > 0 ? ceil_div(V, FV) * FN : 0; }

static int fused_check_args(const void* xt, const void* bmat_p, const void* v_template, const void* a, const void* w_idx,
                            const void* w_val, const void* verts, int num_joints, int M, int V, int kp, int mp, int np) {
    if (!xt || !bmat_p || !v_template || !a || !w_idx || !w_val || !verts) return bad_arg("hps_smpl_mesh_fused: null pointer");
    if (kp <= 0 || kp % 2 != 0) return bad_arg("hps_smpl_mesh_fused: kp must be positive and even");
    if (num_joints < 1 || num_joints > 32) return bad_arg("hps_smpl_mesh_fused: num_joints must be 1..32");
    if (M <= 0 || V <= 0) return 1;
    if (mp % FM != 0 || mp < ceil_div(M, FM) * FM) return bad_arg("hps_smpl_mesh_fused: mp must be a multiple of 64 covering M");
    if (np != hps_smpl_mesh_fused_np(V)) return bad_arg("hps_smpl_mesh_fused: np must be hps_smpl_mesh_fused_np(V)");
    return HPS_OK;
}

extern "C" int hps_smpl_mesh_fused(const float* xt, const float* bmat_p, const float* v_template, const float* a,
                                   const int32_t* w_idx, const float* w_val, int K, int num_joints, const float* transl,
                                   float* verts, int M, int V, int kp, int mp, int np, hps_stream_t stream) {
    const int rc = fused_check_args(xt, bmat_p, v_template, a, w_idx, w_val, verts, num_joints, M, V, kp, mp, np);
    if (rc != HPS_OK) return rc > 0 ? HPS_OK : rc;
    hipStream_t s = (hipStream_t)stream;
    switch (K) {
        case 4: return launch_fused<4>(xt, bmat_p, v_template, a, w_idx, w_val, num_joints, transl, verts, M, V, kp, mp, np, s);
        case 8: return launch_fused<8>(xt, bmat_p, v_template, a, w_idx, w_val, num_joints, transl, verts, M, V, kp, mp, np, s);
        case 12: return launch_fused<12>(xt, bmat_p, v_template, a, w_idx, w_val, num_joints, transl, verts, M, V, kp, mp, np, s);
        default: set_error("hps_smpl_mesh_fused: K=%d unsupported (4 with any joint count; 8, 12 with 24 joints); use "
                           "hps_smpl_blend + hps_smpl_lbs", K); return HPS_E_UNSUPPORTED;
    }
}

extern "C" int hps_smpl_mesh_fused_picks(const float* xt, const float* bmat_p, const float* v_template, const float* a,
                                         const int32_t* w_idx, const float* w_val, int K, int num_joints, const float* transl,
                                         float* verts, int M, int V, int kp, int mp, int np, const int32_t* pick_slot, float* picked,
                                         int n_picked, hps_stream_t stream) {
    if (!pick_slot || !picked || n_picked <= 0) return bad_arg("hps_smpl_mesh_fused_picks: pick_slot / picked / n_picked");
    const int rc = fused_check_args(xt, bmat_p, v_template, a, w_idx, w_val, verts, num_joints, M, V, kp, mp, np);
    if (rc != HPS_OK) return rc > 0 ? HPS_OK : rc;
    if (K != 4) { set_error("hps_smpl_mesh_fused_picks: K = %d (the side output exists for K = 4 only)", K); return HPS_E_UNSUPPORTED; }
    return launch_fused<4>(xt, bmat_p, v_template, a, w_idx, w_val, num_joints, transl, verts, M, V, kp, mp, np, (hipStream_t)stream,
                           pick_slot, picked, n_picked);
}

extern "C" int hps_smpl_mesh_fused_shared_shape(const float* xt_pose, const float* bmat_p_pose, const float* v_shaped,
                                                const int32_t* mesh_row, const int32_t* group_rows, const float* a,
                                                const int32_t* w_idx, const float* w_val, int K, int num_joints, float* verts, int M,
                                                int V, int kp, int mp, int np, const int32_t* pick_slot, float* picked,
                                                int n_picked, hps_stream_t stream) {
    if (!mesh_row || !group_rows || !pick_slot || !picked || n_picked <= 0)
        return bad_arg("hps_smpl_mesh_fused_shared_shape: mesh_row / group_rows / pick_slot / picked / n_picked");
    const int rc = fused_check_args(xt_pose, bmat_p_pose, v_shaped, a, w_idx, w_val, verts, num_joints, M, V, kp, mp, np);
    if (rc != HPS_OK) return rc > 0 ? HPS_OK : rc;
    if (K != 4) { set_error("hps_smpl_mesh_fused_shared_shape: K = %d (exists for K = 4 only)", K); return HPS_E_UNSUPPORTED; }
    return launch_fused<4>(xt_pose, bmat_p_pose, v_shaped, a, w_idx, w_val, num_joints, nullptr, verts, M, V, kp, mp, np,
                           (hipStream_t)stream, pick_slot, picked, n_picked, mesh_row, group_rows);
}

namespace hps {
__global__ __launch_bounds__(256) void v_shaped_kernel(const float* __restrict__ betas, int nb, const float* __restrict__ shape_rows, int ld,
                                                       const float* __restrict__ v_template, float* __restrict__ v_shaped, int n3) {
    const int n = blockIdx.x * 256 + threadIdx.x, r = blockIdx.y;
    if (n >= n3) return;
    float acc = 0.0f;
    for (int l = 0; l < nb; ++l) acc = __builtin_fmaf(betas[r * nb + l], shape_rows[(size_t)l * ld + n], acc);
    v_shaped[(size_t)r * n3 + n] = v_template[n] + acc;
}
}

extern "C" int hps_smpl_v_shaped(const float* betas, int num_betas, const float* shape_rows, int ld, const float* v_template,
                                 float* v_shaped, int R, int V, hps_stream_t stream) {
    if (!betas || !shape_rows || !v_template || !v_shaped) return bad_arg("hps_smpl_v_shaped: null pointer");
    if (num_betas < 0 || ld < 3 * V) return bad_arg("hps_smpl_v_shaped: num_betas >= 0 and ld >= 3 V required");
    if (R <= 0 || V <= 0) return HPS_OK;
    if (R > 65535) return bad_arg("hps_smpl_v_shaped: at most 65535 shapes per call");
    hipLaunchKernelGGL(hps::v_shaped_kernel, dim3(ceil_div(3 * V, 256), R), dim3(256), 0, (hipStream_t)stream, betas, num_betas, shape_rows, ld,
                       v_template, v_shaped, 3 * V);
    return check_launch("hps_smpl_v_shaped");
}

#ifdef HPS_DEV_BUILD
extern "C" int hps_dev_mesh_stages(int stages) {
    g_mesh_stages = stages;
    return HPS_OK;
}
extern "C" int hps_dev_mesh_lds_floor(int bytes) {
    g_mesh_lds_floor = bytes > 0 ? (size_t)bytes : 0;
    return HPS_OK;
}

extern "C" int hps_dev_mesh_fused(const float* xt, const float* bmat_p, const float* v_template, const float* a,
                                  const int32_t* w_idx, const float* w_val, int K, int num_joints, const float* transl,
                                  float* verts, int M, int V, int kp, int mp, int np, int ablate, hps_stream_t stream) {
    const int rc = fused_check_args(xt, bmat_p, v_template, a, w_idx, w_val, verts, num_joints, M, V, kp, mp, np);
    if (rc != HPS_OK) return rc > 0 ? HPS_OK : rc;
    if (K != 4) return bad_arg("hps_dev_mesh_fused: K = 4 only");
    hipStream_t s = (hipStream_t)stream;
    switch (ablate) {
        case 0: return launch_fused<4, 0>(xt, bmat_p, v_template, a, w_idx, w_val, num_joints, transl, verts, M, V, kp, mp, np, s);
        case 1: return launch_fused<4, 1>(xt, bmat_p, v_template, a, w_idx, w_val, num_joints, transl, verts, M, V, kp, mp, np, s);
        case 2: return launch_fused<4, 2>(xt, bmat_p, v_template, a, w_idx, w_val, num_joints, transl, verts, M, V, kp, mp, np, s);
        case 3: return launch_fused<4, 3>(xt, bmat_p, v_template, a, w_idx, w_val, num_joints, transl, verts, M, V, kp, mp, np, s);
        case 4: return launch_fused<4, 4>(xt, bmat_p, v_template, a, w_idx, w_val, num_joints, transl, verts, M, V, kp, mp, np, s);
        case 5: return launch_fused<4, 5>(xt, bmat_p, v_template, a, w_idx, w_val, num_joints, transl, verts, M, V, kp, mp, np, s);
        default: return bad_arg("hps_dev_mesh_fused: ablate 0..5");
    }
}
#endif
```

hierarchicalprobabilistic3dhuman_amd/poseMF_shapeGaussian_net.py:

```python
import os

import torch
from torch import nn
from torch.distributions import Normal

from . import _capi
from .device_state import DeviceStateModule
from .resnet import resnet18
from .rigid_transform_utils import rotmat_to_rot6d
from .sharding import effective_cpus


_SVD_THREADS = max(2, min(16, effective_cpus() // (2 * max(1, int(os.environ.get("LOCAL_WORLD_SIZE", "1"))))))


def _host_svd_packed(f_host, usv_host):
    n = f_host.shape[0]
    assert f_host.is_contiguous() and usv_host.is_contiguous() and not f_host.is_cuda
    _capi.call("hps_host_svd3_packed", _capi._P(f_host.data_ptr()), _capi._P(usv_host.data_ptr()), n, _SVD_THREADS)


def immediate_parents_to_all_parents(immediate_parents):
    all_parents = {}
    for smpl_idx in range(1, len(immediate_parents)):
        joint, parent = smpl_idx - 1, immediate_parents[smpl_idx] - 1
        all_parents[joint] = [parent] + all_parents[parent] if parent >= 0 else []
    return all_parents


class _RefinedHead:

    def __init__(self, net, p, feats, pose_U, pose_S, pose_V):
        self.net, self.p = net, p
        self.feats, self.pose_U = feats.detach(), pose_U.detach()
        self.ptrs = (pose_U.data_ptr(), pose_S.data_ptr(), pose_V.data_ptr())
        self.result = None

    def get(self):
        if self.result is None:
            self.result = self.net._refine(self.p, self.feats, self.pose_U)
            self.feats = self.pose_U = None
        return self.result


class _HeadFunction(torch.autograd.Function):

    @staticmethod
    def forward(ctx, net, p, feats, *params):
        outs = net._head(feats, p)
        pose_F, pose_U, pose_S, pose_V, mode, loc, scale, glob, cam = outs
        ctx.net, ctx.p = net, p
        ctx.save_for_backward(feats, pose_U, scale, *params)
        ctx.refined = None
        if net.differentiable_factors:
            ctx.refined = _RefinedHead(net, p, feats, pose_U, pose_S, pose_V)
        else:
            ctx.mark_non_differentiable(pose_U, pose_V)
        ctx.set_materialize_grads(False)
        return outs

    @staticmethod
    @torch.autograd.function.once_differentiable
    def backward(ctx, g_F, g_U, g_S, g_V, g_mode, g_loc, g_scale, g_glob, g_cam):
        feats, pose_U, scale = ctx.saved_tensors[:3]
        need = ctx.needs_input_grad
        g_feats, g_params = ctx.net._head_backward(ctx.p, feats, pose_U, scale, g_F, g_S, g_mode, g_loc, g_scale, g_glob, g_cam,
                                                   want_feats=need[2], want_params=any(need[3:]), g_U=g_U, g_V=g_V, refined=ctx.refined)
        if g_params is None:
            return (None, None, g_feats) + (None,) * len(need[3:])
        return (None, None, g_feats) + tuple(g if n else None for g, n in zip(g_params, need[3:]))


class PoseMFShapeGaussianNet(DeviceStateModule):
    SWITCHES = ("latency_mode", "svd_mode", "svd_flavor", "composite_head")

    def __init__(self, smpl_parents, config):
        super().__init__()
        self.config = config
        self.parents_dict = immediate_parents_to_all_parents(smpl_parents)
        self.num_joints = len(self.parents_dict)
        self.num_pose_params = self.num_joints * 9
        self.num_shape_params = config.MODEL.NUM_SMPL_BETAS
        self.num_glob_params = 6
        self.num_cam_params = 3
        self.register_buffer("init_glob", rotmat_to_rot6d(torch.eye(3)[None, :].float()))
        self.register_buffer("init_cam", torch.tensor([0.9, 0.0, 0.0]).float())

        if config.MODEL.NUM_RESNET_LAYERS != 18:
            raise NotImplementedError("only the ResNet-18 encoder of the released model is implemented")
        self.image_encoder = resnet18(in_channels=config.MODEL.NUM_IN_CHANNELS, pretrained=False)
        num_image_features, fc1_dim = 512, 512
        embed_dim = config.MODEL.EMBED_DIM

        self.activation = nn.ELU()
        self.fc1 = nn.Linear(num_image_features, fc1_dim)
        self.fc_shape = nn.Linear(fc1_dim, self.num_shape_params * 2)
        self.fc_glob = nn.Linear(fc1_dim, self.num_glob_params)
        self.fc_cam = nn.Linear(fc1_dim, self.num_cam_params)
        self.fc_embed = nn.Linear(num_image_features + self.num_shape_params * 2 + self.num_glob_params
                                  + self.num_cam_params, embed_dim)
        self.fc_pose = nn.ModuleList()
        for joint in range(self.num_joints):
            in_dim = embed_dim + len(self.parents_dict[joint]) * (9 + 3 + 9)
            self.fc_pose.append(nn.Sequential(nn.Linear(in_dim, embed_dim // 2), self.activation,
                                              nn.Linear(embed_dim // 2, 9)))
        depth = [len(self.parents_dict[j]) for j in range(self.num_joints)]
        self.levels = [[j for j in range(self.num_joints) if depth[j] == d] for d in range(max(depth) + 1)]
        self._pinned_bufs = {}
        self.composite_head = True
        self.svd_mode = "device"
        self.svd_flavor = None
        self.latency_mode = False
        self.differentiable_factors = False
        self._track_versions = False

    def set_latency_mode(self, on=True):
        self.latency_mode = bool(on)
        self.image_encoder.set_latency_mode(on)

    def set_batchnorm_training(self, on=True):
        self.image_encoder.set_batchnorm_training(on)

    def set_differentiable_factors(self, on=True):
        self.differentiable_factors = bool(on)

    def _flavor(self):
        return _capi.svd_flavor() if self.svd_flavor is None else int(self.svd_flavor)

    def __getstate__(self):
        state = super().__getstate__()
        state["_pinned_bufs"] = {}
        return state

    def _pinned(self, name, numel):
        stream = torch.cuda.current_stream()
        key = (name, stream.cuda_stream)
        buf = self._pinned_bufs.get(key)
        if buf is None or buf.numel() < numel:
            if buf is not None:
                stream.synchronize()
            buf = torch.empty(max(numel, 1024), dtype=torch.float32, pin_memory=True)
            self._pinned_bufs[key] = buf
        return buf[:numel]

    def prepare(self):
        dev = self.fc1.weight.device
        t = lambda w: w.detach().float().t().contiguous()
        c = lambda w: w.detach().float().contiguous()
        nsh, ng, nc = self.num_shape_params * 2, self.num_glob_params, self.num_cam_params
        p = {}
        p["fc1_wt"], p["fc1_b"] = t(self.fc1.weight), c(self.fc1.bias)
        p["sgc_wt"] = t(torch.cat([self.fc_shape.weight, self.fc_glob.weight, self.fc_cam.weight], dim=0))
        p["sgc_b"] = c(torch.cat([self.fc_shape.bias, self.fc_glob.bias, self.fc_cam.bias]))
        p["sgc_add"] = c(torch.cat([torch.zeros(nsh, device=dev), self.init_glob.reshape(-1), self.init_cam.reshape(-1)]))
        p["embed_wt"], p["embed_b"] = t(self.fc_embed.weight), c(self.fc_embed.bias)
        w1t = [t(m[0].weight) for m in self.fc_pose]
        b1 = [c(m[0].bias) for m in self.fc_pose]
        w2 = [c(m[2].weight) for m in self.fc_pose]
        b2 = [c(m[2].bias) for m in self.fc_pose]
        p["keep"] = (w1t, b1, w2, b2)
        ptrs = lambda ts: torch.tensor([x.data_ptr() for x in ts], dtype=torch.int64, device=dev)
        p["w1t_ptrs"], p["b1_ptrs"], p["w2_ptrs"], p["b2_ptrs"] = ptrs(w1t), ptrs(b1), ptrs(w2), ptrs(b2)
        anc_ptr, anc_idx = [0], []
        for j in range(self.num_joints):
            anc_idx.extend(self.parents_dict[j])
            anc_ptr.append(len(anc_idx))
        p["anc_ptr"] = torch.tensor(anc_ptr, dtype=torch.int32, device=dev)
        p["anc_idx"] = torch.tensor(anc_idx if anc_idx else [0], dtype=torch.int32, device=dev)
        p["levels"] = [torch.tensor(l, dtype=torch.int32, device=dev) for l in self.levels]
        p["level_joints"] = torch.tensor([j for l in self.levels for j in l], dtype=torch.int32, device=dev)
        p["level_sizes_host"] = torch.tensor([len(l) for l in self.levels], dtype=torch.int32)
        p["max_level_size"] = max(len(l) for l in self.levels)
        if self._track_versions:
            p["versions"] = self._head_versions()
        self._prepared = p
        return p

    def _head_params(self):
        ps = [self.fc1.weight, self.fc1.bias, self.fc_shape.weight, self.fc_shape.bias, self.fc_glob.weight, self.fc_glob.bias,
              self.fc_cam.weight, self.fc_cam.bias, self.fc_embed.weight, self.fc_embed.bias]
        for m in self.fc_pose:
            ps += [m[0].weight, m[0].bias, m[2].weight, m[2].bias]
        return ps

    def _head_versions(self):
        return tuple(w._version for w in self._head_params())

    def _prepare_backward(self, p):
        q = p.get("bwd")
        if q is not None:
            return q
        dev = self.fc1.weight.device
        c = lambda w: w.detach().float().contiguous()
        i32 = lambda v: torch.tensor(v if v else [0], dtype=torch.int32, device=dev)
        nj, embed_dim = self.num_joints, self.config.MODEL.EMBED_DIM
        desc_ptr, desc_joint, desc_pos = [0], [], []
        for a in range(nj):
            for d in range(nj):
                if a in self.parents_dict[d]:
                    desc_joint.append(d)
                    desc_pos.append(self.parents_dict[d].index(a))
            desc_ptr.append(len(desc_joint))
        in_off = [0]
        for j in range(nj):
            in_off.append(in_off[-1] + embed_dim + 21 * len(self.parents_dict[j]))
        q = dict(fc1_w=c(self.fc1.weight), embed_w=c(self.fc_embed.weight),
                 sgc_w=c(torch.cat([self.fc_shape.weight, self.fc_glob.weight, self.fc_cam.weight], dim=0)),
                 desc_ptr=i32(desc_ptr), desc_joint=i32(desc_joint), desc_pos=i32(desc_pos), in_off=i32(in_off),
                 in_off_host=in_off, total_in=in_off[-1])
        p["bwd"] = q
        return q

    def _refine(self, p, feats, pose_U):
        B, dev = feats.shape[0], feats.device
        nj, embed_dim = self.num_joints, self.config.MODEL.EMBED_DIM
        nt = 2 * self.num_shape_params + self.num_glob_params + self.num_cam_params
        nf, hidden = feats.shape[1], p["fc1_wt"].shape[1]
        P, VP, s = _capi.ptr, _capi._P, _capi.stream()
        f32 = dict(device=dev, dtype=torch.float32)
        f64 = dict(device=dev, dtype=torch.float64)
        D = lambda t: _capi.ptr(t, torch.float64)
        delta = float(self.config.MODEL.DELTA_I_WEIGHT) if self.config.MODEL.DELTA_I else 0.0
        x_f, sgc_f, embed_f = torch.empty(B, hidden, **f32), torch.empty(B, nt, **f32), torch.empty(B, embed_dim, **f32)
        x_d, sgc_d, embed_d = torch.empty(B, hidden, **f64), torch.empty(B, nt, **f64), torch.empty(B, embed_dim, **f64)
        Up_d, Sp_d, mode_d = torch.empty(B, nj, 9, **f64), torch.empty(B, nj, 3, **f64), torch.empty(B, nj, 9, **f64)
        U_d, S_d, V_d = torch.empty(B, nj, 9, **f64), torch.empty(B, nj, 3, **f64), torch.empty(B, nj, 9, **f64)
        _capi.call("hps_head_forward_refine", P(feats), nf, P(p["fc1_wt"]), P(p["fc1_b"]), P(p["sgc_wt"]), P(p["sgc_b"]), P(p["sgc_add"]),
                   P(p["embed_wt"]), P(p["embed_b"]), _capi.iptr(p["level_joints"]), VP(p["level_sizes_host"].data_ptr()),
                   len(p["levels"]), _capi.iptr(p["anc_ptr"]), _capi.iptr(p["anc_idx"]), VP(p["w1t_ptrs"].data_ptr()),
                   VP(p["b1_ptrs"].data_ptr()), VP(p["w2_ptrs"].data_ptr()), VP(p["b2_ptrs"].data_ptr()), delta, P(pose_U), P(x_f),
                   P(sgc_f), P(embed_f), D(x_d), D(sgc_d), D(embed_d), D(Up_d), D(Sp_d), D(mode_d), D(U_d), D(S_d), D(V_d), B, nf, hidden,
                   nt, embed_dim, embed_dim // 2, nj, s)
        return dict(x_f=x_f, sgc_f=sgc_f, embed_f=embed_f, embed_d=embed_d, Up_d=Up_d, Sp_d=Sp_d, mode_d=mode_d, U_d=U_d, S_d=S_d, V_d=V_d)

    def _head_backward(self, p, feats, pose_U, scale, g_F, g_S, g_mode, g_loc, g_scale, g_glob, g_cam, want_feats=True, want_params=True,
                       g_U=None, g_V=None, refined=None):
        q = self._prepare_backward(p)
        B, dev = feats.shape[0], feats.device
        nj, embed_dim = self.num_joints, self.config.MODEL.EMBED_DIM
        nsh, ng, nc = self.num_shape_params, self.num_glob_params, self.num_cam_params
        nt = 2 * nsh + ng + nc
        nf, hidden = feats.shape[1], p["fc1_wt"].shape[1]
        P, VP, s = _capi.ptr, _capi._P, _capi.stream()
        f32 = dict(device=dev, dtype=torch.float32)
        G = lambda g: None if g is None else _capi.f32c(g)
        g_F, g_S, g_mode, g_loc, g_scale, g_glob, g_cam = G(g_F), G(g_S), G(g_mode), G(g_loc), G(g_scale), G(g_glob), G(g_cam)
        g_U, g_V = G(g_U), G(g_V)
        tail = embed_dim // 2 + 9 * (embed_dim // 2) + 9
        D = lambda t: _capi.ptr(t, torch.float64)
        r = refined.get() if refined is not None else self._refine(p, feats, pose_U)
        x_f, sgc_f, embed_f, embed_d = r["x_f"], r["sgc_f"], r["embed_f"], r["embed_d"]
        Up_d, Sp_d, mode_d, U_d, S_d, V_d = r["Up_d"], r["Sp_d"], r["mode_d"], r["U_d"], r["S_d"], r["V_d"]
        g_embed = torch.empty(B, embed_dim, **f32)
        g_pose = torch.empty((embed_dim // 2) * q["total_in"] + nj * tail, **f32) if want_params else None
        ws = torch.empty(_capi.query_workspace(_capi.WS_HEAD_LEVELS_BWD, B, q["total_in"], nj) // 4, **f32)
        _capi.call("hps_head_pose_levels_backward_factors", D(embed_d), embed_dim, embed_dim // 2, _capi.iptr(p["level_joints"]),
                   VP(p["level_sizes_host"].data_ptr()), len(p["levels"]), _capi.iptr(p["anc_ptr"]), _capi.iptr(p["anc_idx"]),
                   _capi.iptr(q["desc_ptr"]), _capi.iptr(q["desc_joint"]), _capi.iptr(q["desc_pos"]), _capi.iptr(q["in_off"]),
                   VP(p["w1t_ptrs"].data_ptr()), VP(p["b1_ptrs"].data_ptr()), VP(p["w2_ptrs"].data_ptr()), D(Up_d), D(Sp_d),
                   D(mode_d), D(U_d), D(S_d), D(V_d), P(g_F), P(g_S), P(g_mode), P(g_U), P(g_V), P(g_embed), P(g_pose), P(ws), B, nj,
                   q["total_in"], s)
        E = lambda *shape: torch.empty(*shape, **f32) if want_params else None
        g_feats = torch.empty(B, nf, **f32) if want_feats else None
        g_fc1_w, g_fc1_b = E(hidden, nf), E(hidden)
        g_sgc_w, g_sgc_b = E(nt, hidden), E(nt)
        g_embed_w, g_embed_b = E(embed_dim, nf + nt), E(embed_dim)
        ws2 = torch.empty(_capi.query_workspace(_capi.WS_HEAD_TRUNK_BWD, B, nf + hidden + embed_dim, nt) // 4, **f32)
        _capi.call("hps_head_trunk_backward", P(feats), nf, P(x_f), P(sgc_f), P(embed_f), P(scale), P(q["fc1_w"]), P(q["sgc_w"]),
                   P(q["embed_w"]), P(g_embed), P(g_loc), P(g_scale), P(g_glob), P(g_cam), P(g_feats), P(g_fc1_w), P(g_fc1_b),
                   P(g_sgc_w), P(g_sgc_b), P(g_embed_w), P(g_embed_b), P(ws2), B, nf, hidden, nsh, ng, nc, embed_dim, s)
        if not want_params:
            return g_feats, None
        a, b = 2 * nsh, 2 * nsh + ng
        grads = [g_fc1_w, g_fc1_b, g_sgc_w[:a], g_sgc_b[:a], g_sgc_w[a:b], g_sgc_b[a:b], g_sgc_w[b:], g_sgc_b[b:], g_embed_w, g_embed_b]
        hid = embed_dim // 2
        for j in range(nj):
            o = hid * q["in_off_host"][j] + j * tail
            in_dim = q["in_off_host"][j + 1] - q["in_off_host"][j]
            grads += [g_pose[o:o + hid * in_dim].view(hid, in_dim), g_pose[o + hid * in_dim:o + hid * in_dim + hid],
                      g_pose[o + hid * in_dim + hid:o + hid * in_dim + hid + 9 * hid].view(9, hid), g_pose[o + hid * in_dim + 10 * hid:o + hid * in_dim + 10 * hid + 9]]
        return g_feats, grads

    def _trunk(self, feats, p):
        embed, loc, scale, glob, cam = self._trunk_launch(feats, p)
        return embed, Normal(loc=loc, scale=scale, validate_args=False), glob, cam

    def _trunk_launch(self, feats, p):
        B, dev = feats.shape[0], feats.device
        nsh, ng, nc = self.num_shape_params * 2, self.num_glob_params, self.num_cam_params
        embed_dim = self.config.MODEL.EMBED_DIM
        P, s = _capi.ptr, _capi.stream()
        f32 = dict(device=dev, dtype=torch.float32)
        nf = feats.shape[1]
        hidden = p["fc1_wt"].shape[1]
        x = torch.empty(B, hidden, **f32)
        sgc = torch.empty(B, nsh + ng + nc, **f32)
        embed = torch.empty(B, embed_dim, **f32)
        shape_mean = torch.empty(B, self.num_shape_params, **f32)
        shape_scale = torch.empty(B, self.num_shape_params, **f32)
        glob = torch.empty(B, ng, **f32)
        cam = torch.empty(B, nc, **f32)
        _capi.call("hps_head_trunk", P(feats), nf, P(p["fc1_wt"]), P(p["fc1_b"]), P(p["sgc_wt"]), P(p["sgc_b"]), P(p["sgc_add"]),
                   P(p["embed_wt"]), P(p["embed_b"]), P(x), P(sgc), P(embed), P(shape_mean), P(shape_scale), P(glob), P(cam), B, nf,
                   hidden, self.num_shape_params, ng, nc, embed_dim, s)
        return embed, shape_mean, shape_scale, glob, cam

    def _pose_buffers(self, B, dev):
        f32 = dict(device=dev, dtype=torch.float32)
        nj = self.num_joints
        return (torch.empty(B, nj, 3, 3, **f32), torch.empty(B, nj, 3, 3, **f32), torch.empty(B, nj, 3, **f32),
                torch.empty(B, nj, 3, 3, **f32), torch.empty(B, nj, 3, 3, **f32), torch.empty(B, nj, 3, **f32),
                torch.empty(B, nj, 3, 3, **f32))

    def forward(self, input, input_feats=None):
        if input_feats is None:
            input_feats = self.image_encoder(input)
        _capi.require_device(input_feats, "input_feats")
        differentiable = torch.is_grad_enabled() and (input_feats.requires_grad or any(w.requires_grad for w in self._head_params()))
        if differentiable:
            self._track_versions = True
        if self._track_versions and self._prepared is not None and self._prepared.get("versions") != self._head_versions():
            self.invalidate()
        p = self._prepared or self.prepare()
        feats = _capi.f32c(input_feats)
        if differentiable:
            outs = _HeadFunction.apply(self, p, feats, *self._head_params())
            refined = outs[1].grad_fn.refined if outs[1].grad_fn is not None else None
            if refined is not None:
                for t in outs[1:4]:
                    t._hps_refined = refined
        else:
            outs = self._head(feats, p)
        pose_F, pose_U, pose_S, pose_V, mode, loc, scale, glob, cam = outs
        return pose_F, pose_U, pose_S, pose_V, mode, Normal(loc=loc, scale=scale, validate_args=False), glob, cam

    def _head(self, feats, p):
        B = feats.shape[0]
        dev = feats.device
        nj = self.num_joints
        embed_dim = self.config.MODEL.EMBED_DIM
        P, s = _capi.ptr, _capi.stream()
        f32 = dict(device=dev, dtype=torch.float32)
        embed, loc, scale, glob, cam = self._trunk_launch(feats, p)

        pose_F, pose_U, pose_S, pose_V, U_proper, S_proper, mode = self._pose_buffers(B, dev)
        delta = float(self.config.MODEL.DELTA_I_WEIGHT) if self.config.MODEL.DELTA_I else 0.0
        stream = torch.cuda.current_stream()
        if self.svd_mode not in ("device", "host"):
            raise ValueError("svd_mode must be 'device' or 'host'")
        device_svd = self.svd_mode == "device"
        if self.composite_head:
            sizes = p["level_sizes_host"]
            max_n = p["max_level_size"]
            VP = _capi._P
            if device_svd:
                f_dev = usv_dev = None
                fh = uh = None
            else:
                n_f = _capi.query_workspace(_capi.WS_HEAD_F, B, max_n) // 4
                n_usv = _capi.query_workspace(_capi.WS_HEAD_USV, B, max_n) // 4
                f_dev = torch.empty(n_f, **f32)
                usv_dev = torch.empty(n_usv, **f32)
                fh, uh = VP(self._pinned("f", n_f).data_ptr()), VP(self._pinned("usv", n_usv).data_ptr())
            _capi.call("hps_head_pose_levels", P(embed), embed_dim, embed_dim // 2, _capi.iptr(p["level_joints"]),
                       VP(sizes.data_ptr()), len(p["levels"]), _capi.iptr(p["anc_ptr"]), _capi.iptr(p["anc_idx"]),
                       VP(p["w1t_ptrs"].data_ptr()), VP(p["b1_ptrs"].data_ptr()), VP(p["w2_ptrs"].data_ptr()),
                       VP(p["b2_ptrs"].data_ptr()), P(U_proper), P(S_proper), P(mode), delta, P(pose_F), P(pose_U), P(pose_S),
                       P(pose_V), P(f_dev), P(usv_dev), fh, uh, B, nj, _SVD_THREADS,
                       ((_capi.SVD_DEVICE_FMA if self._flavor() == _capi.SVD_ROUNDING_FMA else _capi.SVD_DEVICE) |
                        (_capi.HEAD_WIDE_WORKGROUPS if self.latency_mode else 0)) if device_svd else _capi.SVD_HOST, s)
            return pose_F, pose_U, pose_S, pose_V, mode, loc, scale, glob, cam
        for lvl in p["levels"]:
            n_level = lvl.numel()
            if device_svd:
                _capi.call("hps_head_joint_level_svd", P(embed), embed_dim, embed_dim // 2, _capi.iptr(lvl), n_level,
                           _capi.iptr(p["anc_ptr"]), _capi.iptr(p["anc_idx"]),
                           _capi._P(p["w1t_ptrs"].data_ptr()), _capi._P(p["b1_ptrs"].data_ptr()),
                           _capi._P(p["w2_ptrs"].data_ptr()), _capi._P(p["b2_ptrs"].data_ptr()),
                           P(U_proper), P(S_proper), P(mode), delta, P(pose_F), P(pose_U), P(pose_S), P(pose_V), B, nj,
                           self._flavor() | (_capi.HEAD_WIDE_WORKGROUPS if self.latency_mode else 0), s)
                continue
            f_level = torch.empty(B, n_level, 3, 3, **f32)
            _capi.call("hps_head_joint_level", P(embed), embed_dim, embed_dim // 2, _capi.iptr(lvl), n_level,
                       _capi.iptr(p["anc_ptr"]), _capi.iptr(p["anc_idx"]),
                       _capi._P(p["w1t_ptrs"].data_ptr()), _capi._P(p["b1_ptrs"].data_ptr()),
                       _capi._P(p["w2_ptrs"].data_ptr()), _capi._P(p["b2_ptrs"].data_ptr()),
                       P(U_proper), P(S_proper), P(mode), delta, P(pose_F), P(f_level), B, nj, s)
            f_host = self._pinned("f", B * n_level * 9).view(B * n_level, 3, 3)
            f_host.copy_(f_level.view(B * n_level, 3, 3), non_blocking=True)
            stream.synchronize()
            usv_host = self._pinned("usv", B * n_level * 21).view(B * n_level, 21)
            _host_svd_packed(f_host, usv_host)
            usv = torch.empty(B, n_level, 21, **f32)
            usv.view(B * n_level, 21).copy_(usv_host, non_blocking=True)
            _capi.call("hps_head_svd_finish", P(usv), _capi.iptr(lvl), n_level, P(pose_U), P(pose_S), P(pose_V),
                       P(U_proper), P(S_proper), P(mode), B, nj, s)
        return pose_F, pose_U, pose_S, pose_V, mode, loc, scale, glob, cam
```

include/hps.h:

```cpp
#ifndef HPS_H_
#define HPS_H_

#include <stddef.h>
#include <stdint.h>

#ifdef __cplusplus
extern "C" {
#endif
#pragma GCC visibility push(default)

typedef void* hps_stream_t;


#define HPS_OK 0
#define HPS_E_BADARG (-1)
#define HPS_E_UNSUPPORTED (-2)

#define HPS_SVD_HOST 0
#define HPS_SVD_DEVICE 1
#define HPS_SVD_DEVICE_FMA 2

#define HPS_SVD_ROUNDING_REFERENCE 0
#define HPS_SVD_ROUNDING_FMA 1
#define HPS_HEAD_WIDE_WORKGROUPS 0x100

#define HPS_ACT_NONE 0
#define HPS_ACT_ELU 1
#define HPS_ACT_RELU 2

int hps_version(void);
const char* hps_last_error(void);

int hps_stream_create_cu_partition(int first_cu, int num_cus, hps_stream_t* stream_out);
int hps_stream_destroy(hps_stream_t stream);

enum { HPS_WS_CONV_SPLITK = 0, HPS_WS_SMPL_MP = 1, HPS_WS_SMPL_XT = 2, HPS_WS_SMPL_A = 3, HPS_WS_SMPL_VPOSED = 4,
       HPS_WS_HEAD_F = 5, HPS_WS_HEAD_USV = 6, HPS_WS_MF_LOSS = 8, HPS_WS_SMPL_LBS_BWD = 9, HPS_WS_SMPL_BLEND_BWD = 10,
       HPS_WS_HEAD_LEVELS_BWD = 11, HPS_WS_HEAD_TRUNK_BWD = 12, HPS_WS_SEG_BBOX = 13 };
int64_t hps_query_workspace(int what, int64_t d0, int64_t d1, int64_t d2);


int hps_smpl_pose_prep(const float* glob, const float* body, int is_rotmat, const float* betas,
                       int num_betas, const float* j_template, const float* j_shapedirs,
                       const int32_t* parents, const int32_t* depth, int num_joints, float* xt,
                       int kp, int mp, float* a, float* j_posed, float* rot_out, int M,
                       hps_stream_t stream);

int hps_smpl_blend(const float* xt, const float* bmat, const float* v_template, float* v_posed,
                   int M, int N, int kp, int mp, int np, int ld_out, hps_stream_t stream);

int hps_smpl_lbs(const float* v_posed, int ld_vposed, const float* a, const int32_t* w_idx,
                 const float* w_val, int K, int num_joints, const float* transl, float* verts, int M,
                 int V, hps_stream_t stream);

int hps_smpl_mesh_fused(const float* xt, const float* bmat_p, const float* v_template, const float* a,
                        const int32_t* w_idx, const float* w_val, int K, int num_joints, const float* transl,
                        float* verts, int M, int V, int kp, int mp, int np, hps_stream_t stream);
int hps_smpl_mesh_fused_picks(const float* xt, const float* bmat_p, const float* v_template, const float* a,
                              const int32_t* w_idx, const float* w_val, int K, int num_joints, const float* transl,
                              float* verts, int M, int V, int kp, int mp, int np, const int32_t* pick_slot, float* picked,
                              int n_picked, hps_stream_t stream);
int hps_smpl_mesh_fused_shared_shape(const float* xt_pose, const float* bmat_p_pose, const float* v_shaped,
                                     const int32_t* mesh_row, const int32_t* group_rows, const float* a,
                                     const int32_t* w_idx, const float* w_val, int K, int num_joints, float* verts, int M,
                                     int V, int kp, int mp, int np, const int32_t* pick_slot, float* picked,
                                     int n_picked, hps_stream_t stream);
int hps_smpl_v_shaped(const float* betas, int num_betas, const float* shape_rows, int ld, const float* v_template,
                      float* v_shaped, int R, int V, hps_stream_t stream);
size_t hps_smpl_split_bf16x3_bytes(int rows, int cols);
int hps_smpl_split_bf16x3_mesh_tile(void);
int hps_smpl_split_bf16x3(const float* src, int rows, int ld, int cols, int tile_cols, void* dst, hps_stream_t stream);
int hps_smpl_mesh_fused_shared_shape_bf16x3(const void* xsplit, const void* bsplit, const float* v_shaped, const int32_t* mesh_row,
                                            const int32_t* group_rows, const float* a, const int32_t* w_idx, const float* w_val,
                                            int K, int num_joints, float* verts, int M, int V, int rows, int mp,
                                            const int32_t* pick_slot, float* picked, int n_picked, hps_stream_t stream);
int hps_smpl_mesh_fused_np(int V);

int hps_joints_and_uncertainty(const float* picked, const float* j_posed, const int32_t* csr_ptr, const int32_t* csr_slot,
                               const float* csr_val, int n_rows, int num_joints, const float* transl, float* joints, int M,
                               int n_picked, const float* verts_samples, float* unc, int B, int N, int V, hps_stream_t stream);

int hps_smpl_joints(const float* verts, const float* j_posed, const int32_t* csr_ptr,
                    const int32_t* csr_col, const float* csr_val, int n_rows, int num_joints,
                    const float* transl, float* joints, int M, int V, hps_stream_t stream);


int hps_smpl_lbs_backward(float* v_posed, int ld_vposed, const float* a, const int32_t* w_idx, const float* w_val, int K,
                          int num_joints, const float* g_verts, const float* g_joints, int n_rows, const int32_t* csrt_ptr,
                          const int32_t* csrt_row, const float* csrt_val, float* g_a, float* g_transl, float* workspace, int M,
                          int V, hps_stream_t stream);

int hps_smpl_blend_backward(const float* bmat, const float* g_vposed, float* g_xt, float* workspace, int M, int kp, int mp,
                            int np, int ld_g, hps_stream_t stream);

int hps_smpl_pose_prep_backward(const float* glob, const float* body, int is_rotmat, const float* betas, int num_betas,
                                const float* j_template, const float* j_shapedirs, const int32_t* parents, const int32_t* depth,
                                int num_joints, const float* g_a, const float* g_joints, int n_rows, const float* g_xt, int mp,
                                float* g_glob, float* g_body, float* g_betas, int M, hps_stream_t stream);

int hps_vertex_uncertainty(const float* verts, float* unc, int B, int N, int V, hps_stream_t stream);


int hps_mf_sample(const float* pose_u, const float* pose_s, const float* pose_v,
                  const float* bingham_a, const float* acg_override, int C, int num_joints, int num_samples, int n_prop,
                  float b, float m_star,
                  const float* eps, const float* w, const int32_t* draw_idx, uint64_t seed,
                  int64_t call_offset, const uint64_t* seed_dev, int max_rounds, float* r_out, float* quat_out,
                  int32_t* accepted, hps_stream_t stream);

int hps_mf_sample_keep_quat(const float* pose_u, const float* pose_s, const float* pose_v, int C, int num_joints, int num_samples,
                            int n_prop, float b, float m_star, const float* eps, const float* w, const int32_t* draw_idx,
                            uint64_t seed, int64_t call_offset, int max_rounds, float* r_out, float* quat_out, int32_t* accepted,
                            hps_stream_t stream);

int hps_mf_sample_backward(const float* pose_u, const float* pose_s, const float* pose_v, const double* pose_u_d,
                           const double* pose_s_d, const double* pose_v_d, const float* quat, const float* g_r, int C, int num_joints,
                           int num_samples, float b, float* g_pose_u, float* g_pose_s, float* g_pose_v, hps_stream_t stream);

int hps_infer_assemble(const float* mode, const float* glob_rotmats, const float* loc, const float* betas_samples,
                       float* body, float* glob_all, float* betas_all, int B, int N, int num_body_joints,
                       int num_betas, hps_stream_t stream);

int hps_quat_to_rotmat(const float* quat, float* rotmat, int n, hps_stream_t stream);
int hps_rot6d_to_rotmat(const float* x6, float* rotmat, int n, hps_stream_t stream);
int hps_rot6d_to_rotmat_backward(const float* x6, const float* g_rotmat, float* g_x6, int n, hps_stream_t stream);
int hps_batch_rodrigues(const float* aa, float* rotmat, int n, hps_stream_t stream);


int hps_linear(const float* x, int ldx, const float* wt, const float* bias, const float* addend,
               float* out, int ldo, int B, int K, int N, int act, hps_stream_t stream);

int hps_head_trunk(const float* feats, int ldf, const float* fc1_wt, const float* fc1_b, const float* sgc_wt,
                   const float* sgc_b, const float* sgc_add, const float* embed_wt, const float* embed_b, float* x_ws,
                   float* sgc_out, float* embed, float* shape_loc, float* shape_scale, float* glob, float* cam, int B,
                   int num_feats, int hidden, int num_shape, int num_glob, int num_cam, int embed_dim, hps_stream_t stream);

int hps_head_joint_level(const float* embed, int embed_dim, int hidden, const int32_t* joint_ids,
                         int n_level, const int32_t* anc_ptr, const int32_t* anc_idx,
                         const float* const* w1t_ptrs, const float* const* b1_ptrs,
                         const float* const* w2_ptrs, const float* const* b2_ptrs,
                         const float* u_proper, const float* s_proper, const float* mode,
                         float delta_i_weight, float* pose_f, float* f_level, int B,
                         int num_body_joints, hps_stream_t stream);

int hps_head_joint_level_svd(const float* embed, int embed_dim, int hidden, const int32_t* joint_ids,
                             int n_level, const int32_t* anc_ptr, const int32_t* anc_idx,
                             const float* const* w1t_ptrs, const float* const* b1_ptrs,
                             const float* const* w2_ptrs, const float* const* b2_ptrs, float* u_proper,
                             float* s_proper, float* mode, float delta_i_weight, float* pose_f, float* pose_u,
                             float* pose_s, float* pose_v, int B, int num_body_joints, int svd_flavor,
                             hps_stream_t stream);

int hps_svd3_packed(const float* f, float* usv, int n, int svd_flavor, hps_stream_t stream);

int hps_host_svd3_emulated(const float* f_host, float* usv_host, int n, int svd_flavor);

int hps_host_svd_flavor(void);

int hps_host_svd3_packed(const float* f_host, float* usv_host, int n, int num_threads);
int hps_host_bind_lapack(const char* library_path);

int hps_head_svd_finish(const float* usv_level, const int32_t* joint_ids, int n_level,
                        float* pose_u, float* pose_s, float* pose_v, float* u_proper,
                        float* s_proper, float* mode, int B, int num_body_joints,
                        hps_stream_t stream);


int hps_conv2d_bn_act_pad(const float* x, const float* wn, const float* scale, const float* shift,
                          const float* residual, float* y, int B, int H, int W, int ipad, int Cin, int Cout,
                          int KH, int KW, int stride, int pad, int opad, int relu, int row_mode, int variant,
                          int ksplit, float* splitk_ws, hps_stream_t stream);

int hps_conv2d_bn_act_pad_down(const float* x, const float* wn, const float* scale, const float* shift, float* y,
                               const float* wn_down, const float* scale_down, const float* shift_down, float* y_down,
                               int B, int H, int W, int ipad, int Cin, int Cout, int KH, int KW, int stride, int pad,
                               int opad, int relu, int variant, int ksplit, float* splitk_ws, hps_stream_t stream);

int hps_conv3x3_winograd(const float* x, const float* u, const float* scale, const float* shift,
                         const float* residual, float* y, int B, int H, int W, int ipad, int Cin, int Cout,
                         int opad, int relu, float* splitk_ws, hps_stream_t stream);
size_t hps_conv3x3_winograd_workspace(int B, int H, int W, int Cin, int Cout);

size_t hps_stem_phase_frames_bytes(int B, int H, int W);
int hps_stem_phase_split(const float* x, float* frames, int B, int C, int H, int W, hps_stream_t stream);
int hps_proxy_rep_phase_frames(const float* edge, const float* joints2d, const float* visib, float* frames, int B, int K, int H,
                               int W, float std, hps_stream_t stream);
int hps_stem_winograd(const float* frames, const float* u, const float* scale, const float* shift, float* y, int B, int H,
                      int W, int opad, int relu, hps_stream_t stream);
size_t hps_stem_pool_side_bytes(int B, int H, int W);
int hps_stem_winograd_pooled(const float* frames, const float* u, const float* scale, const float* shift, float* pooled, float* side,
                             int B, int H, int W, int opad, int relu, hps_stream_t stream);
int hps_stem_winograd_pooled_nchw(const float* x, const float* u, const float* scale, const float* shift, float* pooled, float* side,
                                  int B, int H, int W, int opad, int relu, hps_stream_t stream);

enum { HPS_ENC_RELAYOUT = 0, HPS_ENC_CONV = 1, HPS_ENC_MAXPOOL = 2, HPS_ENC_AVGPOOL = 3, HPS_ENC_CONV_WINOGRAD = 4,
       HPS_ENC_STEM_SPLIT = 5, HPS_ENC_STEM_WINOGRAD = 6,
       HPS_ENC_RELAYOUT_GENERIC = 7 ,
       HPS_ENC_STEM_WINOGRAD_POOLED = 8, HPS_ENC_STEM_WINOGRAD_POOLED_NCHW = 9,
       HPS_ENC_CONV_DOWN = 10  };
typedef struct hps_enc_op {
    int kind;
    const float* x;
    const float* w;
    const float* scale;
    const float* shift;
    const float* residual;
    float* y;
    float* splitk_ws;
    int B, H, W, ipad, Cin, Cout, KH, KW, stride, pad, opad, relu, row_mode, variant, ksplit;
    const float* w_down;
    const float* scale_down;
    const float* shift_down;
    float* y_down;
} hps_enc_op;

int hps_sizeof_enc_op(void);

int hps_encoder_run(const hps_enc_op* ops, int n_ops, hps_stream_t stream);

int hps_head_pose_levels(const float* embed, int embed_dim, int hidden, const int32_t* level_joints,
                         const int32_t* level_sizes_host, int n_levels, const int32_t* anc_ptr,
                         const int32_t* anc_idx, const float* const* w1t_ptrs, const float* const* b1_ptrs,
                         const float* const* w2_ptrs, const float* const* b2_ptrs, float* u_proper,
                         float* s_proper, float* mode, float delta_i_weight, float* pose_f, float* pose_u,
                         float* pose_s, float* pose_v, float* f_level_dev, float* usv_level_dev,
                         float* f_host_pinned, float* usv_host_pinned, int B, int num_body_joints,
                         int svd_threads, int svd_mode, hps_stream_t stream);


int hps_head_forward_refine(const float* feats, int ldf, const float* fc1_wt, const float* fc1_b, const float* sgc_wt,
                            const float* sgc_b, const float* sgc_add, const float* embed_wt, const float* embed_b,
                            const int32_t* level_joints, const int32_t* level_sizes_host, int n_levels,
                            const int32_t* anc_ptr, const int32_t* anc_idx, const float* const* w1t_ptrs,
                            const float* const* b1_ptrs, const float* const* w2_ptrs, const float* const* b2_ptrs,
                            float delta_i_weight, const float* pose_u_pin, float* x_f, float* sgc_f, float* embed_f,
                            double* x_d, double* sgc_d, double* embed_d, double* u_proper, double* s_proper, double* mode,
                            double* pose_u, double* pose_s, double* pose_v, int B, int num_feats, int hidden_trunk,
                            int num_sgc, int embed_dim, int hidden, int num_body_joints, hps_stream_t stream);

int hps_head_pose_levels_backward(const double* embed, int embed_dim, int hidden, const int32_t* level_joints,
                                  const int32_t* level_sizes_host, int n_levels, const int32_t* anc_ptr,
                                  const int32_t* anc_idx, const int32_t* desc_ptr, const int32_t* desc_joint,
                                  const int32_t* desc_pos, const int32_t* in_off, const float* const* w1t_ptrs,
                                  const float* const* b1_ptrs, const float* const* w2_ptrs, const double* u_proper,
                                  const double* s_proper, const double* mode, const double* pose_u, const double* pose_s,
                                  const double* pose_v, const float* g_pose_f, const float* g_pose_s, const float* g_mode,
                                  float* g_embed, float* g_fc_pose, float* workspace, int B, int num_body_joints,
                                  int total_in, hps_stream_t stream);

int hps_head_pose_levels_backward_factors(const double* embed, int embed_dim, int hidden, const int32_t* level_joints,
                                          const int32_t* level_sizes_host, int n_levels, const int32_t* anc_ptr,
                                          const int32_t* anc_idx, const int32_t* desc_ptr, const int32_t* desc_joint,
                                          const int32_t* desc_pos, const int32_t* in_off, const float* const* w1t_ptrs,
                                          const float* const* b1_ptrs, const float* const* w2_ptrs, const double* u_proper,
                                          const double* s_proper, const double* mode, const double* pose_u, const double* pose_s,
                                          const double* pose_v, const float* g_pose_f, const float* g_pose_s, const float* g_mode,
                                          const float* g_pose_u, const float* g_pose_v, float* g_embed, float* g_fc_pose,
                                          float* workspace, int B, int num_body_joints, int total_in, hps_stream_t stream);

int hps_head_trunk_backward(const float* feats, int ldf, const float* x, const float* sgc, const float* embed,
                            const float* shape_scale, const float* fc1_w, const float* sgc_w, const float* embed_w,
                            const float* g_embed, const float* g_loc, const float* g_scale, const float* g_glob,
                            const float* g_cam, float* g_feats, float* g_fc1_w, float* g_fc1_b, float* g_sgc_w,
                            float* g_sgc_b, float* g_embed_w, float* g_embed_b, float* workspace, int B, int num_feats,
                            int hidden, int num_shape, int num_glob, int num_cam, int embed_dim, hps_stream_t stream);

int hps_nchw_to_padded_nhwc(const float* x, float* y, int B, int C, int H, int W, int P, hps_stream_t stream);

int hps_nchw_to_padded_nhwc_generic(const float* x, float* y, int B, int C, int CP, int H, int W, int WF, int P,
                                    hps_stream_t stream);

int hps_maxpool3x3s2_pad(const float* x, float* y, int B, int H, int W, int C, int opad, hps_stream_t stream);

int hps_global_avgpool_pad(const float* x, float* y, int B, int H, int W, int C, int P, hps_stream_t stream);


int hps_conv_wgrad(const float* x, const float* g, float* G, float* workspace, int B, int H, int W, int ipad, int Cx, int Cin,
                   int Cout, int KH, int KW, int stride, int pad, int gpad, hps_stream_t stream);
int hps_conv_wgrad_slice_pixels(int Ho, int Wo);
size_t hps_conv_wgrad_workspace(int B, int H, int W, int Cin, int Cout, int KH, int KW, int stride, int pad);

int hps_conv_dgrad(const float* g, const float* wt, const float* other, float* dx, int B, int H, int W, int Cin, int Cout, int KH,
                   int KW, int stride, int pad, int gpad, int dpad, int Cdx, hps_stream_t stream);

int hps_relu_gate_pad(float* g, const float* y, double* workspace, float* sums, int B, int H, int W, int C, int gpad, int ypad,
                      hps_stream_t stream);
size_t hps_relu_gate_workspace(int B, int H, int W, int C);

int hps_maxpool3x3s2_backward(const float* x, const float* gpool, float* dx, int B, int H, int W, int C, int gpad, hps_stream_t stream);

int hps_global_avgpool_backward(const float* gfeat, float* gframe, int B, int H, int W, int C, int P, hps_stream_t stream);


int hps_bn_batch_stats(const float* z, double* workspace, double* mean, double* var, int B, int H, int W, int C, int pad,
                       hps_stream_t stream);
size_t hps_bn_batch_stats_workspace(int B, int H, int W, int C);

int hps_bn_train_fold(const double* mean, const double* var, double* invstd, const float* gamma, const float* beta, double eps,
                      double momentum, long long n, float* scale, float* shift, float* running_mean, float* running_var,
                      long long* num_batches_tracked, int C, hps_stream_t stream);

int hps_bn_apply_act_pad(const float* z, const float* scale, const float* shift, const float* residual, float* y, int B, int H, int W,
                         int C, int zpad, int ypad, int relu, hps_stream_t stream);

int hps_bn_train_backward_sums(float* g, const float* z, const float* y, const double* mean, const double* invstd, double* workspace,
                               double* sums, int B, int H, int W, int C, int gpad, int zpad, int ypad, hps_stream_t stream);
size_t hps_bn_train_backward_sums_workspace(int B, int H, int W, int C);

int hps_bn_train_backward_dz(const float* g, const float* z, const double* mean, const double* invstd, const float* gamma,
                             const double* sums, float* dz, int B, int H, int W, int C, int gpad, int zpad, int dpad, hps_stream_t stream);


int hps_canny_edges(const float* img, const float* gauss_taps_host, int gauss_size, float* blurred,
                    float* grad_mag, float* grad_ori, float* thr_mag, float* thin, float* thr_thin,
                    int B, int C, int H, int W, float threshold, int nms, hps_stream_t stream);

int hps_canny_edge_map(const float* img, const float* gauss_taps_host, int gauss_size, float* edge_out,
                       int64_t edge_batch_stride, int B, int C, int H, int W, float threshold, int nms, hps_stream_t stream);

int hps_proxy_rep(const float* edge, const float* joints2d, const float* visib, float* out, int B,
                  int K, int H, int W, float std, hps_stream_t stream);

int hps_heatmaps_to_joints2d(const float* heatmaps, float* joints2d, float* visib, int BK, int H, int W,
                             float eps, hps_stream_t stream);

int hps_sample_joints2d_error(const float* joints, const int32_t* coco_map, int n_joints_all,
                              const float* in_j2d, const float* in_vis, const float* cam, float img_wh,
                              float* err, int N, int K, hps_stream_t stream);

#define HPS_TRAIN_PLAN_WORDS 84
#define HPS_TRAIN_NUM_JOINTS 17
#define HPS_TRAIN_NUM_PART_COUNTS 8

int hps_seg_bbox_affine(const float* part, int64_t part_batch_stride, const int32_t* plan, int B, int H, int W, int out_wh,
                        float orig_scale_factor, int32_t* ws, float* affine, float* theta, int32_t* status, int32_t* part_counts,
                        hps_stream_t stream);

#define HPS_TRAIN_RESAMPLE 1
#define HPS_TRAIN_COUNT 128
#define HPS_TRAIN_COUNT14 256
#define HPS_TRAIN_CROP_CLASS_MASK 4
#define HPS_TRAIN_CLASS_MASK 2
#define HPS_TRAIN_SEG_OCCLUDE 8
#define HPS_TRAIN_BACKGROUND 16
#define HPS_TRAIN_RGB_OCCLUDE 32
#define HPS_TRAIN_RGB_NOISE 64
#define HPS_TRAIN_ALL_STAGES 511

int hps_train_crop_augment(const float* part, int64_t part_batch_stride, const float* rgb, const float* background,
                           const float* theta, const int32_t* plan, int B, int H, int W, int D, int stages, float* rgb_out,
                           int32_t* part_counts, float* part_crop, float* part_aug, hps_stream_t stream);

#define HPS_TRAIN_J_PRE_VIS 1
#define HPS_TRAIN_J_AFFINE 2
#define HPS_TRAIN_J_POST_VIS 4
#define HPS_TRAIN_J_OCCLUDED 8
#define HPS_TRAIN_J_SEG_AUG 16
#define HPS_TRAIN_J_RGB_AUG 32
#define HPS_TRAIN_J_ALL_STAGES 63

int hps_train_joints2d(const float* joints2d, const uint8_t* vis_in, const float* affine, const int32_t* part_counts,
                       const int32_t* plan, int B, int K, float img_wh, int pixel_count_threshold, int stages, float* joints_target,
                       float* joints_input, float* vis, uint8_t* vis_u8, hps_stream_t stream);


int hps_pointset_errors(const float* pred, const float* target, int S, int group, int P, int mode,
                        double* stats_ws, float* xf_ws, double* err_sum, float* transformed,
                        hps_stream_t stream);

int hps_sums_f64(const float* const* xs, const int64_t* ns, const int32_t* take_abs, int count, double first,
                 double* partial_ws, double* out, double* accumulate, hps_stream_t stream);


int hps_mf_log_norm_const(const float* S, int n, float* log_c, const float* grad_log_c, float* grad_S, hps_stream_t stream);

int hps_mf_nll(const float* F, const float* U, const float* S, const float* V, const float* R, int n, double overreg, float* nll,
               const float* grad_nll, float* grad_F, float* grad_S, hps_stream_t stream);

#define HPS_MF_REDUCTION_MEAN 0
#define HPS_MF_REDUCTION_SUM 1
typedef struct hps_mf_loss_args {
    int struct_bytes;
    int reduction;
    int64_t n_pose;
    int64_t shape_B, n_shape;
    int64_t j2d_B, Ns, K;
    int64_t n_glob, n_verts, n_joints3d;
    double img_wh, overreg;
    double weights[6];
    const float *pose_F, *pose_U, *pose_S, *pose_V;
    const float *shape_loc, *shape_scale, *joints2d, *glob_rotmats, *verts, *joints3d;
    const float *t_pose_rotmats, *t_shape, *t_joints2d;
    const uint8_t* t_joints2d_vis;
    const float *t_glob_rotmats, *t_verts, *t_joints3d;
    float *g_pose_F, *g_pose_S, *g_shape_loc, *g_shape_scale;
    float *g_joints2d, *g_glob_rotmats, *g_verts, *g_joints3d;
} hps_mf_loss_args;

int hps_mf_loss_forward(const hps_mf_loss_args* args, void* workspace, float* total, hps_stream_t stream);
int hps_mf_loss_backward(const hps_mf_loss_args* args, const void* workspace, const float* grad_total, hps_stream_t stream);

#pragma GCC visibility pop
#ifdef __cplusplus
}
#endif
#endif
```

Baseline: 22570.

## Size head joint-level LDS by max ancestor count and raise linear occupancy

The joint-level head kernels now size their LDS from the actual maximum number of ancestors instead of the total joint count, which shrinks the per-workgroup LDS footprint. More workgroups can then be resident and the wide 1024-thread variant is allowed more often. The linear kernel's batch tile TB drops from 8 to 4 and it gets a launch-bounds occupancy hint. A dev-only mesh launch path is added behind a flag. Risks are a smaller batch tile giving less weight reuse in the linear kernel, and an early-exit guard for joints that exceed max_anc.

```diff
diff --git a/hierarchicalprobabilistic3dhuman_amd/_capi.py b/hierarchicalprobabilistic3dhuman_amd/_capi.py
--- a/hierarchicalprobabilistic3dhuman_amd/_capi.py
+++ b/hierarchicalprobabilistic3dhuman_amd/_capi.py
@@ -46,6 +46,9 @@
     "hps_head_trunk": [_P] + [_I] + [_P] * 14 + [_I] * 7 + [_P],
     "hps_head_joint_level": [_P, _I, _I, _P, _I, _P, _P, _P, _P, _P, _P, _P, _P, _P, _c.c_float, _P, _P, _I, _I, _P],
     "hps_head_joint_level_svd": [_P, _I, _I, _P, _I, _P, _P, _P, _P, _P, _P, _P, _P, _P, _c.c_float, _P, _P, _P, _P, _I, _I, _I, _P],
+    "hps_head_joint_level_anc": [_P, _I, _I, _P, _I, _P, _P, _P, _P, _P, _P, _P, _P, _P, _c.c_float, _P, _P, _I, _I, _I, _P],
+    "hps_head_joint_level_svd_anc": [_P, _I, _I, _P, _I, _P, _P, _P, _P, _P, _P, _P, _P, _P, _c.c_float, _P, _P, _P, _P, _I, _I, _I, _I, _P],
+    "hps_head_lds_bytes": [_I, _I, _I],
     "hps_svd3_packed": [_P, _P, _I, _I, _P],
     "hps_host_svd3_emulated": [_P, _P, _I, _I],
     "hps_host_svd_flavor": [],
@@ -74,6 +77,8 @@
     "hps_encoder_run": [_P, _I, _P],
     "hps_head_pose_levels": [_P, _I, _I, _P, _P, _I, _P, _P, _P, _P, _P, _P, _P, _P, _P, _c.c_float, _P, _P, _P, _P, _P, _P,
                              _P, _P, _I, _I, _I, _I, _P],
+    "hps_head_pose_levels_anc": [_P, _I, _I, _P, _P, _I, _P, _P, _P, _P, _P, _P, _P, _P, _P, _c.c_float, _P, _P, _P, _P, _P, _P,
+                                 _P, _P, _I, _I, _I, _I, _I, _P],
     "hps_nchw_to_padded_nhwc": [_P, _P, _I, _I, _I, _I, _I, _P],
     "hps_nchw_to_padded_nhwc_generic": [_P, _P, _I, _I, _I, _I, _I, _I, _I, _P],
     "hps_maxpool3x3s2_pad": [_P, _P, _I, _I, _I, _I, _I, _P],
@@ -108,7 +113,7 @@
     "hps_train_crop_augment": [_P, _c.c_int64, _P, _P, _P, _P, _I, _I, _I, _I, _I, _P, _P, _P, _P, _P],
     "hps_train_joints2d": [_P, _P, _P, _P, _P, _I, _I, _c.c_float, _I, _I, _P, _P, _P, _P, _P],
 }
-_RESTYPES = {"hps_last_error": _c.c_char_p, "hps_smpl_split_bf16x3_bytes": _c.c_size_t, "hps_query_workspace": _c.c_int64, "hps_conv3x3_winograd_workspace": _c.c_size_t,
+_RESTYPES = {"hps_last_error": _c.c_char_p, "hps_head_lds_bytes": _c.c_size_t, "hps_smpl_split_bf16x3_bytes": _c.c_size_t, "hps_query_workspace": _c.c_int64, "hps_conv3x3_winograd_workspace": _c.c_size_t,
              "hps_stem_phase_frames_bytes": _c.c_size_t, "hps_stem_pool_side_bytes": _c.c_size_t,
              "hps_conv_wgrad_workspace": _c.c_size_t, "hps_relu_gate_workspace": _c.c_size_t,
              "hps_bn_batch_stats_workspace": _c.c_size_t, "hps_bn_train_backward_sums_workspace": _c.c_size_t}
diff --git a/hierarchicalprobabilistic3dhuman_amd/csrc/composite.hip b/hierarchicalprobabilistic3dhuman_amd/csrc/composite.hip
--- a/hierarchicalprobabilistic3dhuman_amd/csrc/composite.hip
+++ b/hierarchicalprobabilistic3dhuman_amd/csrc/composite.hip
@@ -58,14 +58,14 @@
     return HPS_OK;
 }
 
-extern "C" int hps_head_pose_levels(const float* embed, int embed_dim, int hidden, const int32_t* level_joints,
-                                    const int32_t* level_sizes_host, int n_levels, const int32_t* anc_ptr,
-                                    const int32_t* anc_idx, const float* const* w1t_ptrs, const float* const* b1_ptrs,
-                                    const float* const* w2_ptrs, const float* const* b2_ptrs, float* u_proper,
-                                    float* s_proper, float* mode, float delta_i_weight, float* pose_f, float* pose_u,
-                                    float* pose_s, float* pose_v, float* f_level_dev, float* usv_level_dev,
-                                    float* f_host_pinned, float* usv_host_pinned, int B, int num_body_joints,
-                                    int svd_threads, int svd_mode, hps_stream_t stream) {
+extern "C" int hps_head_pose_levels_anc(const float* embed, int embed_dim, int hidden, const int32_t* level_joints,
+                                        const int32_t* level_sizes_host, int n_levels, const int32_t* anc_ptr,
+                                        const int32_t* anc_idx, const float* const* w1t_ptrs, const float* const* b1_ptrs,
+                                        const float* const* w2_ptrs, const float* const* b2_ptrs, float* u_proper,
+                                        float* s_proper, float* mode, float delta_i_weight, float* pose_f, float* pose_u,
+                                        float* pose_s, float* pose_v, float* f_level_dev, float* usv_level_dev,
+                                        float* f_host_pinned, float* usv_host_pinned, int B, int num_body_joints,
+                                        int max_ancestors, int svd_threads, int svd_mode, hps_stream_t stream) {
     if (!embed || !level_joints || !level_sizes_host) return bad_arg("hps_head_pose_levels: null pointer");
     const int wide = svd_mode & HPS_HEAD_WIDE_WORKGROUPS;
     svd_mode &= ~HPS_HEAD_WIDE_WORKGROUPS;
@@ -74,9 +74,10 @@
         int first_d = 0;
         for (int l = 0; l < n_levels; ++l) {
             const int n_level = level_sizes_host[l];
-            const int rc = hps_head_joint_level_svd(embed, embed_dim, hidden, level_joints + first_d, n_level, anc_ptr, anc_idx,
-                                                    w1t_ptrs, b1_ptrs, w2_ptrs, b2_ptrs, u_proper, s_proper, mode, delta_i_weight,
-                                                    pose_f, pose_u, pose_s, pose_v, B, num_body_joints, flavor, stream);
+            const int rc = hps_head_joint_level_svd_anc(embed, embed_dim, hidden, level_joints + first_d, n_level, anc_ptr, anc_idx,
+                                                        w1t_ptrs, b1_ptrs, w2_ptrs, b2_ptrs, u_proper, s_proper, mode, delta_i_weight,
+                                                        pose_f, pose_u, pose_s, pose_v, B, num_body_joints, max_ancestors, flavor,
+                                                        stream);
             if (rc != HPS_OK) return rc;
             first_d += n_level;
         }
@@ -91,9 +92,9 @@
         const int n_level = level_sizes_host[l];
         const int32_t* ids = level_joints + first;
         const size_t count = (size_t)B * n_level;
-        int rc = hps_head_joint_level(embed, embed_dim, hidden, ids, n_level, anc_ptr, anc_idx, w1t_ptrs, b1_ptrs, w2_ptrs,
-                                      b2_ptrs, u_proper, s_proper, mode, delta_i_weight, pose_f, f_level_dev, B,
-                                      num_body_joints, stream);
+        int rc = hps_head_joint_level_anc(embed, embed_dim, hidden, ids, n_level, anc_ptr, anc_idx, w1t_ptrs, b1_ptrs, w2_ptrs,
+                                          b2_ptrs, u_proper, s_proper, mode, delta_i_weight, pose_f, f_level_dev, B,
+                                          num_body_joints, max_ancestors, stream);
         if (rc != HPS_OK) return rc;
         hipError_t e = hipMemcpyAsync(f_host_pinned, f_level_dev, count * 9 * sizeof(float), hipMemcpyDeviceToHost, s);
         if (e == hipSuccess) e = hipStreamSynchronize(s);
@@ -115,3 +116,17 @@
     }
     return HPS_OK;
 }
+
+extern "C" int hps_head_pose_levels(const float* embed, int embed_dim, int hidden, const int32_t* level_joints,
+                                    const int32_t* level_sizes_host, int n_levels, const int32_t* anc_ptr,
+                                    const int32_t* anc_idx, const float* const* w1t_ptrs, const float* const* b1_ptrs,
+                                    const float* const* w2_ptrs, const float* const* b2_ptrs, float* u_proper,
+                                    float* s_proper, float* mode, float delta_i_weight, float* pose_f, float* pose_u,
+                                    float* pose_s, float* pose_v, float* f_level_dev, float* usv_level_dev,
+                                    float* f_host_pinned, float* usv_host_pinned, int B, int num_body_joints,
+                                    int svd_threads, int svd_mode, hps_stream_t stream) {
+    return hps_head_pose_levels_anc(embed, embed_dim, hidden, level_joints, level_sizes_host, n_levels, anc_ptr, anc_idx, w1t_ptrs,
+                                    b1_ptrs, w2_ptrs, b2_ptrs, u_proper, s_proper, mode, delta_i_weight, pose_f, pose_u, pose_s, pose_v,
+                                    f_level_dev, usv_level_dev, f_host_pinned, usv_host_pinned, B, num_body_joints, num_body_joints,
+                                    svd_threads, svd_mode, stream);
+}
diff --git a/hierarchicalprobabilistic3dhuman_amd/csrc/head.hip b/hierarchicalprobabilistic3dhuman_amd/csrc/head.hip
--- a/hierarchicalprobabilistic3dhuman_amd/csrc/head.hip
+++ b/hierarchicalprobabilistic3dhuman_amd/csrc/head.hip
@@ -6,9 +6,11 @@
 __device__ __forceinline__ float elu1(float x) { return x > 0.0f ? x : expm1f(x); }
 
 
-constexpr int TB = 8;
+constexpr int TB = 4;
+constexpr int LINEAR_MAX_K = 1792;
 constexpr int LCOLS = 16;
 constexpr int LKS = 16;
+constexpr int HEAD_WG_PER_CU = 8;
 
 template <int ROWS>
 __device__ __forceinline__ void dot_slice(const float* __restrict__ w, size_t ldw, const float* xs, int k_lo, int k_hi,
@@ -46,7 +48,7 @@
     int nsh, ng, nc;
 };
 
-__global__ __launch_bounds__(256) void linear_kernel(const float* __restrict__ x, int ldx, const float* __restrict__ x2, int ldx2, int K1,
+__global__ __launch_bounds__(256, HEAD_WG_PER_CU) void linear_kernel(const float* __restrict__ x, int ldx, const float* __restrict__ x2, int ldx2, int K1,
                                                      const float* __restrict__ wt,
                                                      const float* __restrict__ bias, const float* __restrict__ addend,
                                                      float* __restrict__ out, int ldo, int B, int K, int N, int act, TrunkSplit split) {
@@ -237,10 +239,12 @@
     const float* const* __restrict__ b1_ptrs, const float* const* __restrict__ w2_ptrs,
     const float* const* __restrict__ b2_ptrs, float* u_proper, float* s_proper,
     float* mode, float delta_i_weight, float* __restrict__ pose_f, float* __restrict__ f_level,
-    float* __restrict__ pose_u, float* __restrict__ pose_s, float* __restrict__ pose_v, int B, int NJ, int svd_flavor) {
+    float* __restrict__ pose_u, float* __restrict__ pose_s, float* __restrict__ pose_v, int B, int NJ, int svd_flavor, int max_anc) {
     __builtin_amdgcn_s_setprio(3);
     extern __shared__ __attribute__((aligned(16))) float smem[];
-    joint_level_body<HID, DEVSVD, NT, TBL>(smem, joint_ids[blockIdx.x], (int)blockIdx.x, (int)gridDim.x, (int)blockIdx.y * TBL, embed,
+    const int joint_id = joint_ids[blockIdx.x];
+    if (anc_ptr[joint_id + 1] - anc_ptr[joint_id] > max_anc) return;
+    joint_level_body<HID, DEVSVD, NT, TBL>(smem, joint_id, (int)blockIdx.x, (int)gridDim.x, (int)blockIdx.y * TBL, embed,
                                            embed_dim, anc_ptr, anc_idx, w1t_ptrs, b1_ptrs, w2_ptrs, b2_ptrs, u_proper, s_proper, mode,
                                            delta_i_weight, pose_f, f_level, pose_u, pose_s, pose_v, B, NJ, svd_flavor);
 }
@@ -322,10 +326,18 @@
 
 using namespace hps;
 
+static size_t linear_lds(int K) { return ((size_t)((K * TB + 3) & ~3) + LKS * TB * LCOLS) * sizeof(float); }
+
+static size_t joint_level_lds(int embed_dim, int max_anc, int nt) {
+    constexpr int TBL = 4;
+    const size_t max_in = (size_t)embed_dim + 21 * (size_t)max_anc;
+    return (((max_in * TBL + 3) & ~(size_t)3) + 128 * TBL + (size_t)(nt / 128) * TBL * 128) * sizeof(float);
+}
+
 static int launch_linear(const char* who, const float* x, int ldx, const float* x2, int ldx2, int K1, const float* wt, const float* bias,
                          const float* addend, float* out, int ldo, int B, int K, int N, int act, TrunkSplit split, hps_stream_t stream) {
-    size_t lds = ((size_t)((K * TB + 3) & ~3) + LKS * TB * LCOLS) * sizeof(float);
-    if (lds > 64 * 1024) { set_error("%s: K=%d too large for the LDS tile", who, K); return HPS_E_UNSUPPORTED; }
+    const size_t lds = linear_lds(K);
+    if (K > LINEAR_MAX_K) { set_error("%s: K=%d too large for the LDS tile", who, K); return HPS_E_UNSUPPORTED; }
     hipLaunchKernelGGL(linear_kernel, dim3(ceil_div(N, LCOLS), ceil_div(B, TB)), dim3(256), lds, (hipStream_t)stream, x,
                        ldx, x2, ldx2, K1, wt, bias, addend, out, ldo, B, K, N, act, split);
     return check_launch(who);
@@ -367,7 +379,7 @@
                               const float* const* b1_ptrs, const float* const* w2_ptrs, const float* const* b2_ptrs,
                               float* u_proper, float* s_proper, float* mode, float delta_i_weight, float* pose_f,
                               float* f_level, float* pose_u, float* pose_s, float* pose_v, int B, int num_body_joints,
-                              int svd_flavor, hps_stream_t stream) {
+                              int max_ancestors, int svd_flavor, hps_stream_t stream) {
     const bool devsvd = pose_u != nullptr;
     const bool wide = devsvd && (svd_flavor & HPS_HEAD_WIDE_WORKGROUPS) != 0;
     svd_flavor &= ~HPS_HEAD_WIDE_WORKGROUPS;
@@ -377,25 +389,25 @@
         !s_proper || !mode || !pose_f || (devsvd && (!pose_s || !pose_v)))
         return bad_arg("hps_head_joint_level: null pointer");
     if (hidden != 128) { set_error("hps_head_joint_level: hidden=%d unsupported (128 = EMBED_DIM/2)", hidden); return HPS_E_UNSUPPORTED; }
+    if (embed_dim <= 0 || num_body_joints <= 0 || max_ancestors < 0 || max_ancestors > num_body_joints)
+        return bad_arg("hps_head_joint_level: embed_dim / num_body_joints / max_ancestors");
     if (B <= 0 || n_level <= 0) return HPS_OK;
-    constexpr int NT = 256, TBL = 4;
-    const int max_in = embed_dim + 21 * num_body_joints;
-    size_t lds = ((size_t)((max_in * TBL + 3) & ~3) + 128 * TBL + (NT / 128) * TBL * 128) * sizeof(float);
+    constexpr int NT = 256, TBL = 4, NTW = 1024;
+    const int max_anc = max_ancestors;
+    const size_t lds = joint_level_lds(embed_dim, max_anc, NT), ldsw = joint_level_lds(embed_dim, max_anc, NTW);
     if (lds > 64 * 1024) { set_error("hps_head_joint_level: embed_dim=%d too large", embed_dim); return HPS_E_UNSUPPORTED; }
-    constexpr int NTW = 1024;
-    const size_t ldsw = ((size_t)((max_in * TBL + 3) & ~3) + 128 * TBL + (NTW / 128) * TBL * 128) * sizeof(float);
     if (wide && ldsw <= 64 * 1024) {
         hipLaunchKernelGGL((joint_level_kernel<128, true, NTW, TBL>), dim3(n_level, ceil_div(B, TBL)), dim3(NTW), ldsw, (hipStream_t)stream,
                            embed, embed_dim, joint_ids, anc_ptr, anc_idx, w1t_ptrs, b1_ptrs, w2_ptrs, b2_ptrs, u_proper,
-                           s_proper, mode, delta_i_weight, pose_f, f_level, pose_u, pose_s, pose_v, B, num_body_joints, svd_flavor);
+                           s_proper, mode, delta_i_weight, pose_f, f_level, pose_u, pose_s, pose_v, B, num_body_joints, svd_flavor, max_anc);
     } else if (devsvd)
         hipLaunchKernelGGL((joint_level_kernel<128, true, NT, TBL>), dim3(n_level, ceil_div(B, TBL)), dim3(NT), lds, (hipStream_t)stream,
                            embed, embed_dim, joint_ids, anc_ptr, anc_idx, w1t_ptrs, b1_ptrs, w2_ptrs, b2_ptrs, u_proper,
-                           s_proper, mode, delta_i_weight, pose_f, f_level, pose_u, pose_s, pose_v, B, num_body_joints, svd_flavor);
+                           s_proper, mode, delta_i_weight, pose_f, f_level, pose_u, pose_s, pose_v, B, num_body_joints, svd_flavor, max_anc);
     else
         hipLaunchKernelGGL((joint_level_kernel<128, false, NT, TBL>), dim3(n_level, ceil_div(B, TBL)), dim3(NT), lds, (hipStream_t)stream,
                            embed, embed_dim, joint_ids, anc_ptr, anc_idx, w1t_ptrs, b1_ptrs, w2_ptrs, b2_ptrs, u_proper,
-                           s_proper, mode, delta_i_weight, pose_f, f_level, pose_u, pose_s, pose_v, B, num_body_joints, svd_flavor);
+                           s_proper, mode, delta_i_weight, pose_f, f_level, pose_u, pose_s, pose_v, B, num_body_joints, svd_flavor, max_anc);
     return check_launch("hps_head_joint_level");
 }
 
@@ -407,7 +419,18 @@
                                     float* f_level, int B, int num_body_joints, hps_stream_t stream) {
     return joint_level_launch(embed, embed_dim, hidden, joint_ids, n_level, anc_ptr, anc_idx, w1t_ptrs, b1_ptrs, w2_ptrs, b2_ptrs,
                               const_cast<float*>(u_proper), const_cast<float*>(s_proper), const_cast<float*>(mode),
-                              delta_i_weight, pose_f, f_level, nullptr, nullptr, nullptr, B, num_body_joints, 0, stream);
+                              delta_i_weight, pose_f, f_level, nullptr, nullptr, nullptr, B, num_body_joints, num_body_joints, 0, stream);
+}
+
+extern "C" int hps_head_joint_level_anc(const float* embed, int embed_dim, int hidden, const int32_t* joint_ids,
+                                        int n_level, const int32_t* anc_ptr, const int32_t* anc_idx,
+                                        const float* const* w1t_ptrs, const float* const* b1_ptrs,
+                                        const float* const* w2_ptrs, const float* const* b2_ptrs, const float* u_proper,
+                                        const float* s_proper, const float* mode, float delta_i_weight, float* pose_f,
+                                        float* f_level, int B, int num_body_joints, int max_ancestors, hps_stream_t stream) {
+    return joint_level_launch(embed, embed_dim, hidden, joint_ids, n_level, anc_ptr, anc_idx, w1t_ptrs, b1_ptrs, w2_ptrs, b2_ptrs,
+                              const_cast<float*>(u_proper), const_cast<float*>(s_proper), const_cast<float*>(mode),
+                              delta_i_weight, pose_f, f_level, nullptr, nullptr, nullptr, B, num_body_joints, max_ancestors, 0, stream);
 }
 
 extern "C" int hps_head_joint_level_svd(const float* embed, int embed_dim, int hidden, const int32_t* joint_ids,
@@ -420,7 +443,29 @@
     if (!pose_u) return bad_arg("hps_head_joint_level_svd: null pointer");
     return joint_level_launch(embed, embed_dim, hidden, joint_ids, n_level, anc_ptr, anc_idx, w1t_ptrs, b1_ptrs, w2_ptrs, b2_ptrs,
                               u_proper, s_proper, mode, delta_i_weight, pose_f, nullptr, pose_u, pose_s, pose_v, B,
-                              num_body_joints, svd_flavor, stream);
+                              num_body_joints, num_body_joints, svd_flavor, stream);
+}
+
+extern "C" int hps_head_joint_level_svd_anc(const float* embed, int embed_dim, int hidden, const int32_t* joint_ids,
+                                            int n_level, const int32_t* anc_ptr, const int32_t* anc_idx,
+                                            const float* const* w1t_ptrs, const float* const* b1_ptrs,
+                                            const float* const* w2_ptrs, const float* const* b2_ptrs, float* u_proper,
+                                            float* s_proper, float* mode, float delta_i_weight, float* pose_f, float* pose_u,
+                                            float* pose_s, float* pose_v, int B, int num_body_joints, int max_ancestors,
+                                            int svd_flavor, hps_stream_t stream) {
+    if (!pose_u) return bad_arg("hps_head_joint_level_svd: null pointer");
+    return joint_level_launch(embed, embed_dim, hidden, joint_ids, n_level, anc_ptr, anc_idx, w1t_ptrs, b1_ptrs, w2_ptrs, b2_ptrs,
+                              u_proper, s_proper, mode, delta_i_weight, pose_f, nullptr, pose_u, pose_s, pose_v, B,
+                              num_body_joints, max_ancestors, svd_flavor, stream);
+}
+
+extern "C" size_t hps_head_lds_bytes(int kernel, int embed_dim_or_k, int max_ancestors) {
+    switch (kernel) {
+        case HPS_HEAD_LDS_LINEAR: return linear_lds(embed_dim_or_k);
+        case HPS_HEAD_LDS_JOINT_LEVEL: return joint_level_lds(embed_dim_or_k, max_ancestors, 256);
+        case HPS_HEAD_LDS_JOINT_LEVEL_WIDE: return joint_level_lds(embed_dim_or_k, max_ancestors, 1024);
+        default: return 0;
+    }
 }
 
 #ifdef HPS_DEV_BUILD
diff --git a/hierarchicalprobabilistic3dhuman_amd/csrc/mesh_epilogue.h b/hierarchicalprobabilistic3dhuman_amd/csrc/mesh_epilogue.h
--- a/hierarchicalprobabilistic3dhuman_amd/csrc/mesh_epilogue.h
+++ b/hierarchicalprobabilistic3dhuman_amd/csrc/mesh_epilogue.h
@@ -39,6 +39,27 @@
 };
 
 template <int K, int MG, bool VS, bool PICK>
+__device__ __forceinline__ void mesh_lane_vertex(MeshLane<K>& L, int m0, int V, const int32_t* __restrict__ w_idx,
+                                                 const float* __restrict__ w_val, const float* __restrict__ v_template,
+                                                 const int32_t* __restrict__ group_rows, const int32_t* __restrict__ pick_slot) {
+#pragma unroll
+    for (int k = 0; k < K; ++k) {
+        L.idx[k] = w_idx[(size_t)L.vc * K + k] * 12;
+        L.w[k] = w_val[(size_t)L.vc * K + k];
+    }
+    const f3* vtp = reinterpret_cast<const f3*>(v_template);
+    if (VS) {
+        const int32_t* gr = group_rows + 3 * __builtin_amdgcn_readfirstlane((m0 + L.wm * 32) >> 5);
+        L.vt = vtp[(size_t)gr[0] * V + L.vc];
+        L.vtb = vtp[(size_t)gr[1] * V + L.vc];
+    } else {
+        L.vt = vtp[L.vc];
+        L.vtb = L.vt;
+    }
+    L.pick = PICK && L.live_v ? pick_slot[L.vc] : -1;
+}
+
+template <int K, int MG, bool VS, bool PICK, bool LATE = false>
 __device__ __forceinline__ MeshLane<K> mesh_lane(int panel, int m0, int V, const int32_t* __restrict__ w_idx,
                                                  const float* __restrict__ w_val, const float* __restrict__ v_template,
                                                  const int32_t* __restrict__ group_rows, const int32_t* __restrict__ pick_slot) {
@@ -53,28 +74,16 @@
     L.v = panel * MESH_PANEL + L.wn * 32 + L.il;
     L.live_v = L.v < V;
     L.vc = L.live_v ? L.v : V - 1;
-#pragma unroll
-    for (int k = 0; k < K; ++k) {
-        L.idx[k] = w_idx[(size_t)L.vc * K + k] * 12;
-        L.w[k] = w_val[(size_t)L.vc * K + k];
-    }
-    const f3* vtp = reinterpret_cast<const f3*>(v_template);
     L.split = 32;
     L.many = false;
     if (VS) {
         const int32_t* gr = group_rows + 3 * __builtin_amdgcn_readfirstlane((m0 + L.wm * 32) >> 5);
-        const int row_a = gr[0], row_b = gr[1];
         L.split = gr[2];
-        L.vt = vtp[(size_t)row_a * V + L.vc];
-        L.vtb = vtp[(size_t)row_b * V + L.vc];
 #pragma unroll
         for (int h = 0; h < MG; ++h) L.many |= group_rows[3 * (m0 / 32 + h) + 2] < 0;
-    } else {
-        L.vt = vtp[L.vc];
-        L.vtb = L.vt;
     }
     L.split_lane = L.split - 4 * L.kl;
-    L.pick = PICK && L.live_v ? pick_slot[L.vc] : -1;
+    if (!LATE) mesh_lane_vertex<K, MG, VS, PICK>(L, m0, V, w_idx, w_val, v_template, group_rows, pick_slot);
     return L;
 }
 
diff --git a/hierarchicalprobabilistic3dhuman_amd/csrc/mesh_fused.hip b/hierarchicalprobabilistic3dhuman_amd/csrc/mesh_fused.hip
--- a/hierarchicalprobabilistic3dhuman_amd/csrc/mesh_fused.hip
+++ b/hierarchicalprobabilistic3dhuman_amd/csrc/mesh_fused.hip
@@ -14,8 +14,8 @@
 constexpr int F_BP = FBK * FN / 256;
 static_assert(F_XP == FW && F_BP % FW == 0, "DMA pieces must divide evenly over the waves");
 
-template <int K, int ABL, int JC, bool HAS_T, int TAIL = FBK / 2, int ST = 2, bool PICK = false, bool VS = false>
-__global__ __launch_bounds__(FT, 4) void mesh_fused_kernel(
+template <int K, int ABL, int JC, bool HAS_T, int TAIL, int ST, bool PICK, bool VS, bool LATE = false>
+__device__ __forceinline__ void mesh_fused_body(
     const float* __restrict__ xt, const float* __restrict__ bmat_p, const float* __restrict__ v_template,
     const float* __restrict__ a, const int32_t* __restrict__ w_idx, const float* __restrict__ w_val, int J,
     const float* __restrict__ transl, f3* __restrict__ verts, int M, int V, int kp, int mp, int np, int tiles_m,
@@ -27,7 +27,7 @@
     int tile_m, panel;
     if (!mesh_block(tiles_m, tiles_m_per_xcd, tile_m, panel)) return;
     const int m0 = tile_m * FM;
-    const MeshLane<K> L = mesh_lane<K, FM / 32, VS, PICK>(panel, m0, V, w_idx, w_val, v_template, group_rows, pick_slot);
+    MeshLane<K> L = mesh_lane<K, FM / 32, VS, PICK, LATE>(panel, m0, V, w_idx, w_val, v_template, group_rows, pick_slot);
     const int lane = L.lane, wave = L.wave, kl = L.kl, il = L.il, wm = L.wm, wn = L.wn;
 
     unsigned b_off[F_BP / FW];
@@ -118,6 +118,7 @@
     for (int c = 0; c + 1 < nchunks; ++c) do_chunk(std::integral_constant<int, FBK / 2>(), c, ABL != 4);
     do_chunk(std::integral_constant<int, TAIL>(), nchunks - 1, false);
 
+    if (LATE) mesh_lane_vertex<K, FM / 32, VS, PICK>(L, m0, V, w_idx, w_val, v_template, group_rows, pick_slot);
     if (ABL == 3) {
         mesh_keep_acc(acc, verts);
         return;
@@ -126,10 +127,37 @@
                                                                                        mesh_row, verts, picked, n_picked);
 }
 
-#ifdef HPS_DEV_BUILD
+#define HPS_MESH_PARAMS                                                                                                            \
+    const float* __restrict__ xt, const float* __restrict__ bmat_p, const float* __restrict__ v_template,                          \
+    const float* __restrict__ a, const int32_t* __restrict__ w_idx, const float* __restrict__ w_val, int J,                        \
+    const float* __restrict__ transl, f3* __restrict__ verts, int M, int V, int kp, int mp, int np, int tiles_m,                   \
+    int tiles_m_per_xcd, const int32_t* __restrict__ pick_slot, f3* __restrict__ picked, int n_picked,                             \
+    const int32_t* __restrict__ mesh_row, const int32_t* __restrict__ group_rows
+#define HPS_MESH_ARGS                                                                                                              \
+    xt, bmat_p, v_template, a, w_idx, w_val, J, transl, verts, M, V, kp, mp, np, tiles_m, tiles_m_per_xcd, pick_slot, picked,      \
+    n_picked, mesh_row, group_rows
+
+template <int K, int ABL, int JC, bool HAS_T, int TAIL = FBK / 2, int ST = 2, bool PICK = false, bool VS = false>
+__global__ __launch_bounds__(FT, 4) void mesh_fused_kernel(HPS_MESH_PARAMS) {
+    mesh_fused_body<K, ABL, JC, HAS_T, TAIL, ST, PICK, VS>(HPS_MESH_ARGS);
+}
+
+constexpr int MESH_VS_REGISTERS = 112;
+template <>
+__global__ __launch_bounds__(FT, 4) __attribute__((amdgpu_num_vgpr(MESH_VS_REGISTERS / 2))) void mesh_fused_kernel<4, 0, 24, false, 8, 2, true, true>(
+    HPS_MESH_PARAMS) {
+    mesh_fused_body<4, 0, 24, false, 8, 2, true, true, true>(HPS_MESH_ARGS);
+}
+
+#ifdef HPS_DEV_BUILD
+__global__ __launch_bounds__(FT, 4) void mesh_fused_free_kernel(HPS_MESH_PARAMS) {
+    mesh_fused_body<4, 0, 24, false, 8, 2, true, true>(HPS_MESH_ARGS);
+}
 static size_t g_mesh_lds_floor = 0;
 static int g_mesh_stages = 0;
 #endif
+#undef HPS_MESH_PARAMS
+#undef HPS_MESH_ARGS
 
 template <int K, int ABL, int JC, bool HAS_T>
 static int launch_fused_cfg(const float* xt, const float* bmat_p, const float* v_template, const float* a, const int32_t* w_idx,
@@ -143,7 +171,7 @@
     const int tiles_m = ceil_div(M, FM), n_panels = ceil_div(V, FV);
     const bool few = tiles_m <= 2
 #ifdef HPS_DEV_BUILD
-                     && g_mesh_stages != 2
+                     && (g_mesh_stages & 0xff) != 2
 #endif
         ;
     const MeshGrid g = mesh_grid(tiles_m, n_panels);
@@ -166,6 +194,15 @@
                 lds = (size_t)4 * max(4 * F_CHUNK_FLOATS, 32 * J * 12);
                 HPS_MESH_LAUNCH(K, ABL, JC, HAS_T, 8, 4, true, true);
             } else {
+#ifdef HPS_DEV_BUILD
+                if (g_mesh_stages & 0x100) {
+                    if (int rc = grant_lds<&mesh_fused_free_kernel>(160 * 1024, "hps_smpl_mesh_fused")) return rc;
+                    hipLaunchKernelGGL(mesh_fused_free_kernel, dim3(g.blocks), dim3(FT), lds, s, xt, bmat_p, v_template, a, w_idx, w_val, J,
+                                       transl, reinterpret_cast<f3*>(verts), M, V, kp, mp, np, tiles_m, g.tiles_m_per_xcd, pick_slot, pk,
+                                       n_picked, mesh_row, group_rows);
+                    return check_launch("hps_smpl_mesh_fused_shared_shape");
+                }
+#endif
                 HPS_MESH_LAUNCH(K, ABL, JC, HAS_T, 8, 2, true, true);
             }
             return check_launch("hps_smpl_mesh_fused_shared_shape");
diff --git a/hierarchicalprobabilistic3dhuman_amd/poseMF_shapeGaussian_net.py b/hierarchicalprobabilistic3dhuman_amd/poseMF_shapeGaussian_net.py
--- a/hierarchicalprobabilistic3dhuman_amd/poseMF_shapeGaussian_net.py
+++ b/hierarchicalprobabilistic3dhuman_amd/poseMF_shapeGaussian_net.py
@@ -171,6 +171,7 @@
         p["level_joints"] = torch.tensor([j for l in self.levels for j in l], dtype=torch.int32, device=dev)
         p["level_sizes_host"] = torch.tensor([len(l) for l in self.levels], dtype=torch.int32)
         p["max_level_size"] = max(len(l) for l in self.levels)
+        p["max_ancestors"] = max(len(self.parents_dict[j]) for j in range(self.num_joints))
         if self._track_versions:
             p["versions"] = self._head_versions()
         self._prepared = p
@@ -362,30 +363,30 @@
                 f_dev = torch.empty(n_f, **f32)
                 usv_dev = torch.empty(n_usv, **f32)
                 fh, uh = VP(self._pinned("f", n_f).data_ptr()), VP(self._pinned("usv", n_usv).data_ptr())
-            _capi.call("hps_head_pose_levels", P(embed), embed_dim, embed_dim // 2, _capi.iptr(p["level_joints"]),
+            _capi.call("hps_head_pose_levels_anc", P(embed), embed_dim, embed_dim // 2, _capi.iptr(p["level_joints"]),
                        VP(sizes.data_ptr()), len(p["levels"]), _capi.iptr(p["anc_ptr"]), _capi.iptr(p["anc_idx"]),
                        VP(p["w1t_ptrs"].data_ptr()), VP(p["b1_ptrs"].data_ptr()), VP(p["w2_ptrs"].data_ptr()),
                        VP(p["b2_ptrs"].data_ptr()), P(U_proper), P(S_proper), P(mode), delta, P(pose_F), P(pose_U), P(pose_S),
-                       P(pose_V), P(f_dev), P(usv_dev), fh, uh, B, nj, _SVD_THREADS,
+                       P(pose_V), P(f_dev), P(usv_dev), fh, uh, B, nj, p["max_ancestors"], _SVD_THREADS,
                        ((_capi.SVD_DEVICE_FMA if self._flavor() == _capi.SVD_ROUNDING_FMA else _capi.SVD_DEVICE) |
                         (_capi.HEAD_WIDE_WORKGROUPS if self.latency_mode else 0)) if device_svd else _capi.SVD_HOST, s)
             return pose_F, pose_U, pose_S, pose_V, mode, loc, scale, glob, cam
         for lvl in p["levels"]:
             n_level = lvl.numel()
             if device_svd:
-                _capi.call("hps_head_joint_level_svd", P(embed), embed_dim, embed_dim // 2, _capi.iptr(lvl), n_level,
+                _capi.call("hps_head_joint_level_svd_anc", P(embed), embed_dim, embed_dim // 2, _capi.iptr(lvl), n_level,
                            _capi.iptr(p["anc_ptr"]), _capi.iptr(p["anc_idx"]),
                            _capi._P(p["w1t_ptrs"].data_ptr()), _capi._P(p["b1_ptrs"].data_ptr()),
                            _capi._P(p["w2_ptrs"].data_ptr()), _capi._P(p["b2_ptrs"].data_ptr()),
                            P(U_proper), P(S_proper), P(mode), delta, P(pose_F), P(pose_U), P(pose_S), P(pose_V), B, nj,
-                           self._flavor() | (_capi.HEAD_WIDE_WORKGROUPS if self.latency_mode else 0), s)
+                           p["max_ancestors"], self._flavor() | (_capi.HEAD_WIDE_WORKGROUPS if self.latency_mode else 0), s)
                 continue
             f_level = torch.empty(B, n_level, 3, 3, **f32)
-            _capi.call("hps_head_joint_level", P(embed), embed_dim, embed_dim // 2, _capi.iptr(lvl), n_level,
+            _capi.call("hps_head_joint_level_anc", P(embed), embed_dim, embed_dim // 2, _capi.iptr(lvl), n_level,
                        _capi.iptr(p["anc_ptr"]), _capi.iptr(p["anc_idx"]),
                        _capi._P(p["w1t_ptrs"].data_ptr()), _capi._P(p["b1_ptrs"].data_ptr()),
                        _capi._P(p["w2_ptrs"].data_ptr()), _capi._P(p["b2_ptrs"].data_ptr()),
-                       P(U_proper), P(S_proper), P(mode), delta, P(pose_F), P(f_level), B, nj, s)
+                       P(U_proper), P(S_proper), P(mode), delta, P(pose_F), P(f_level), B, nj, p["max_ancestors"], s)
             f_host = self._pinned("f", B * n_level * 9).view(B * n_level, 3, 3)
             f_host.copy_(f_level.view(B * n_level, 3, 3), non_blocking=True)
             stream.synchronize()
diff --git a/include/hps.h b/include/hps.h
--- a/include/hps.h
+++ b/include/hps.h
@@ -151,6 +151,26 @@
                              float* pose_s, float* pose_v, int B, int num_body_joints, int svd_flavor,
                              hps_stream_t stream);
 
+int hps_head_joint_level_anc(const float* embed, int embed_dim, int hidden, const int32_t* joint_ids,
+                             int n_level, const int32_t* anc_ptr, const int32_t* anc_idx,
+                             const float* const* w1t_ptrs, const float* const* b1_ptrs,
+                             const float* const* w2_ptrs, const float* const* b2_ptrs,
+                             const float* u_proper, const float* s_proper, const float* mode,
+                             float delta_i_weight, float* pose_f, float* f_level, int B,
+                             int num_body_joints, int max_ancestors, hps_stream_t stream);
+int hps_head_joint_level_svd_anc(const float* embed, int embed_dim, int hidden, const int32_t* joint_ids,
+                                 int n_level, const int32_t* anc_ptr, const int32_t* anc_idx,
+                                 const float* const* w1t_ptrs, const float* const* b1_ptrs,
+                                 const float* const* w2_ptrs, const float* const* b2_ptrs, float* u_proper,
+                                 float* s_proper, float* mode, float delta_i_weight, float* pose_f, float* pose_u,
+                                 float* pose_s, float* pose_v, int B, int num_body_joints, int max_ancestors,
+                                 int svd_flavor, hps_stream_t stream);
+
+#define HPS_HEAD_LDS_LINEAR 0
+#define HPS_HEAD_LDS_JOINT_LEVEL 1
+#define HPS_HEAD_LDS_JOINT_LEVEL_WIDE 2
+size_t hps_head_lds_bytes(int kernel, int dim, int max_ancestors);
+
 int hps_svd3_packed(const float* f, float* usv, int n, int svd_flavor, hps_stream_t stream);
 
 int hps_host_svd3_emulated(const float* f_host, float* usv_host, int n, int svd_flavor);
@@ -226,6 +246,14 @@
                          float* pose_s, float* pose_v, float* f_level_dev, float* usv_level_dev,
                          float* f_host_pinned, float* usv_host_pinned, int B, int num_body_joints,
                          int svd_threads, int svd_mode, hps_stream_t stream);
+int hps_head_pose_levels_anc(const float* embed, int embed_dim, int hidden, const int32_t* level_joints,
+                             const int32_t* level_sizes_host, int n_levels, const int32_t* anc_ptr,
+                             const int32_t* anc_idx, const float* const* w1t_ptrs, const float* const* b1_ptrs,
+                             const float* const* w2_ptrs, const float* const* b2_ptrs, float* u_proper,
+                             float* s_proper, float* mode, float delta_i_weight, float* pose_f, float* pose_u,
+                             float* pose_s, float* pose_v, float* f_level_dev, float* usv_level_dev,
+                             float* f_host_pinned, float* usv_host_pinned, int B, int num_body_joints, int max_ancestors,
+                             int svd_threads, int svd_mode, hps_stream_t stream);
 
 
 int hps_head_forward_refine(const float* feats, int ldf, const float* fc1_wt, const float* fc1_b, const float* sgc_wt,
```

Result: no change. 22670, median of 6 (+0.5%).
